# qiukunlong/seeksv

Measured on AMD Instinct MI355X. Metric: BAM records/sec through getclip+getsv, higher is better.
Workload: dtype i32/u8 (fp64 match-rate compare)

## Files before the change

include/seeksv_hip.h:

```cpp
#ifndef SEEKSV_HIP_H_
#define SEEKSV_HIP_H_

#include <stddef.h>
#include <stdint.h>

#ifdef __cplusplus
extern "C" {
#endif

#define SSV_ABI_VERSION 9

typedef enum {
	SSV_OK = 0,
	SSV_E_NODEVICE = -1,
	SSV_E_HIP = -2,
	SSV_E_ARG = -3,
	SSV_E_STATE = -4,
	SSV_E_NOMEM = -5,
	SSV_E_RANGE = -6
} ssv_status;

typedef enum {
	SSV_MEM_HOST = 0,
	SSV_MEM_DEVICE = 1,
	SSV_MEM_PERSISTENT = 2
} ssv_mem;

typedef struct {
	int32_t tid, pos;
	uint16_t flag;
	uint8_t mapq;
	uint8_t xc;
	uint16_t n_cigar;
	uint16_t pad;
	int32_t l_qseq, mtid, mpos, isize;
	uint32_t cigar_off;
	uint32_t cigar_head[5];
	uint64_t seq_off;
} ssv_record;

#define SSV_NO_SEQ UINT64_MAX
typedef struct {
	int64_t n;
	int32_t mem;
	int32_t max_ref_span;
	const int32_t *tid;
	const int32_t *pos;
	const uint16_t *flag;
	const uint8_t *mapq;
	const uint16_t *n_cigar;
	const int32_t *l_qseq;
	const int32_t *mtid;
	const int32_t *mpos;
	const int32_t *isize;
	const uint32_t *cigar_off;
	const uint32_t *cigar;
	const uint8_t *xc;
	const uint64_t *seq_off;
	const uint8_t *seqqual;
	int64_t n_cigar_total;
	int64_t seqqual_bytes;
	const ssv_record *rec;
	const uint8_t *cigar_ends;
	const struct ssv_tid_run *tid_runs;
	int64_t n_tid_runs;
} ssv_batch_t;

typedef struct ssv_tid_run { int64_t first; int32_t tid; int32_t pad; } ssv_tid_run;

typedef struct ssv_ctx ssv_ctx;


int ssv_ctx_create(int device, ssv_ctx **out);
void ssv_ctx_destroy(ssv_ctx *ctx);
int ssv_sync(ssv_ctx *ctx);
const char *ssv_last_error(const ssv_ctx *ctx);
int ssv_abi_version(void);
int ssv_device_count(void);
void *ssv_stream(ssv_ctx *ctx);

int ssv_host_alloc(size_t bytes, void **p);
int ssv_host_free(void *p);
int ssv_host_register(void *p, size_t bytes);
int ssv_host_unregister(void *p);
int ssv_host_bind_near(void *p, size_t bytes, int device);
int ssv_batch_prefetch(ssv_ctx *ctx, const ssv_batch_t *b);
int ssv_batch_prefetch_drop(ssv_ctx *ctx);

int ssv_batch_retain(ssv_ctx *ctx, const ssv_batch_t *device_batch, ssv_batch_t *out);
int ssv_batch_release(ssv_ctx *ctx, ssv_batch_t *retained);


typedef struct {
	double match_rate;
	int32_t min_mapq;
	int32_t save_low_quality;
	int32_t use_ownership;
	int32_t initial_last_tid;
	int32_t own_lo_tid, own_lo_pos;
	int32_t own_hi_tid, own_hi_pos;
} ssv_clip_params;

int ssv_clip_begin(ssv_ctx *ctx, const ssv_clip_params *p);
int ssv_clip_scan(ssv_ctx *ctx, const ssv_batch_t *b);
int ssv_clip_scan_range(ssv_ctx *ctx, const ssv_batch_t *b, int64_t rec_begin, int64_t rec_end);
int ssv_clip_event_count(ssv_ctx *ctx, int64_t *n_events);

typedef struct {
	int32_t tid;
	uint8_t side;
	uint8_t pad[3];
	int64_t first;
} ssv_table_run;

typedef struct {
	int64_t n_clusters;
	int64_t n_events;
	const int32_t *tid;
	const int32_t *pos;
	const uint8_t *side;
	const int32_t *support;
	const int32_t *left_len;
	const int32_t *right_len;
	const uint8_t *qual_missing;
	const uint64_t *str_off;
	const uint8_t *str;
	const uint64_t *cigar_off;
	const int32_t *n_cigar;
	const uint32_t *cigar;
	int32_t seq_packed;
	int32_t qual_bits;
	uint8_t qual_alphabet[64];
	int32_t format;
	int32_t base_bits;
	int32_t len_bytes, support_bytes, ncig_bytes;
	int32_t qual_group;
	const void *c_len;
	const void *c_support;
	const void *c_ncig;
	const uint8_t *c_flags;
	const ssv_table_run *runs;
	int64_t n_runs;
	const uint64_t *base_exc;
	int64_t n_base_exc;
	uint64_t str_bytes;
	uint64_t cigar_ops;
	int64_t support_sum;
	const void *c_cigar;
	int32_t cigar_bytes, pad4;
} ssv_cluster_table;

int ssv_clip_table_format(ssv_ctx *ctx, int format);
int ssv_clip_table_expand(ssv_ctx *ctx, ssv_cluster_table *t, int32_t n_threads);
typedef struct {
	int32_t narrow, pad;
	uint64_t total;
	uint64_t rows, flags, cigar, runs, base_exc, pos_esc, str;
} ssv_table_wire;
int ssv_clip_table_wire_bytes(ssv_ctx *ctx, const ssv_cluster_table *t, ssv_table_wire *out);
uint64_t ssv_table_block_bytes3(int64_t n_bases, int32_t base_bits, int32_t qual_bits);
uint64_t ssv_table_block_bytes3g(int64_t n_bases, int32_t base_bits, int32_t qual_bits, int32_t qual_group);
uint64_t ssv_table_block_bytes(int32_t left_len, int32_t right_len);

int ssv_clip_cluster(ssv_ctx *ctx, ssv_cluster_table *out);
int ssv_clip_cluster_async(ssv_ctx *ctx, int64_t *n_clusters, int64_t *n_events);
int ssv_clip_table_wait(ssv_ctx *ctx, ssv_cluster_table *out);
int ssv_clip_table_wait_prev(ssv_ctx *ctx, ssv_cluster_table *out);


int ssv_isize_begin(ssv_ctx *ctx, int32_t min_mapq, int64_t max_pairs);
int ssv_isize_accumulate(ssv_ctx *ctx, const ssv_batch_t *b, int32_t *done);
int ssv_isize_finish(ssv_ctx *ctx, int64_t *n_pairs, int32_t *mean, int32_t *sd);


typedef struct {
	int32_t up_tid;
	int32_t down_tid;
	int32_t up_pos;
	int32_t down_pos;
	int32_t beg;
	int32_t end;
	uint8_t up_strand;
	uint8_t down_strand;
	uint8_t pad[2];
} ssv_junction;

typedef struct {
	int32_t tid;
	int32_t beg;
	int32_t end;
} ssv_interval;

typedef struct {
	const ssv_junction *junctions;
	int64_t n_junctions;
	int32_t mean, sd, times;
	int32_t disc_min_mapq;
	const ssv_interval *windows;
	int64_t n_windows;
	int32_t depth_min_mapq;
	int32_t n_targets;
	const int32_t *target_len;
} ssv_getsv_params;

int ssv_getsv_begin(ssv_ctx *ctx, const ssv_getsv_params *p);
int ssv_getsv_scan(ssv_ctx *ctx, const ssv_batch_t *b);
int ssv_getsv_prime(ssv_ctx *ctx, const ssv_batch_t *b, int32_t *sufficient);
int ssv_getsv_finish(ssv_ctx *ctx, int32_t *counts,
                     const ssv_interval *ranges, int64_t n_ranges, uint64_t *range_sum,
                     const ssv_interval *points, int64_t n_points, int32_t *point_depth,
                     int32_t *max_depth);

typedef struct ssv_group ssv_group;
int ssv_group_create(ssv_ctx **ctxs, int n, ssv_group **out);
void ssv_group_destroy(ssv_group *g);
int ssv_group_uses_rccl(const ssv_group *g);
int ssv_group_allgather(ssv_group *g, int rank, const void *send, size_t bytes, void *recv);


typedef struct {
	uint64_t c_off;
	uint32_t c_len;
	uint32_t u_len;
} ssv_bgzf_block;

typedef struct {
	int64_t n_records;
	uint64_t inflated_bytes;
	uint64_t tail_offset;
	uint32_t repaired_blocks;
	int32_t last_tid;
	const uint8_t *unmapped_raw;
	uint64_t unmapped_bytes;
	uint32_t n_tid_runs;
	const uint32_t *tid_run_index;
	const int32_t *tid_run_tid;
} ssv_bamdec_info;

int ssv_bamdec_begin(ssv_ctx *ctx, int32_t n_targets, uint64_t first_record_offset);
int ssv_bamdec_target_lens(ssv_ctx *ctx, const int32_t *lens);
int ssv_bamdec_limit(ssv_ctx *ctx, uint64_t inflated_bytes);
int ssv_bamdec_expect(ssv_ctx *ctx, uint64_t inflated_bytes);
int ssv_bamdec_verify_crc(ssv_ctx *ctx, int on);
int ssv_bamdec_any_order(ssv_ctx *ctx, int on);
int ssv_bamdec_prev_tid(ssv_ctx *ctx, int32_t tid);
int ssv_bamdec_staging(ssv_ctx *ctx, int which, size_t bytes, void **host_ptr);
int ssv_bamdec_prefetch(ssv_ctx *ctx, const void *comp, size_t comp_bytes);
int ssv_bamdec_prefetch_drop(ssv_ctx *ctx);
int ssv_bamdec_decode(ssv_ctx *ctx, const void *comp, size_t comp_bytes, const ssv_bgzf_block *blocks, int64_t n_blocks, int keep_all_seq, ssv_batch_t *out);
int ssv_bamdec_last(ssv_ctx *ctx, ssv_bamdec_info *info);

typedef struct {
	int32_t mem;
	int32_t pad;
	int64_t bias;
	const char *base;
	const uint64_t *off;
	int64_t bytes;
} ssv_names_t;
int ssv_bamdec_names(ssv_ctx *ctx, ssv_names_t *out);
typedef struct {
	int32_t n_targets;
	int32_t pad;
	const char *const *target_names;
	uint64_t first_line;
} ssv_samdec_params;

typedef struct {
	int64_t n_records;
	uint64_t lines_consumed;
	uint64_t carried_bytes;
	uint64_t refused_line;
	const char *refused_reason;
} ssv_samdec_info;

int ssv_samdec_begin(ssv_ctx *ctx, const ssv_samdec_params *p);
int ssv_samdec_prefetch(ssv_ctx *ctx, const void *text, size_t bytes);
int ssv_samdec_decode(ssv_ctx *ctx, const void *text, size_t bytes, int mem, int last, ssv_batch_t *out);
int ssv_samdec_names(ssv_ctx *ctx, ssv_names_t *out);
int ssv_samdec_last(ssv_ctx *ctx, ssv_samdec_info *info);
int ssv_samdec_sorted(ssv_ctx *ctx, int keep_all_seq);
int ssv_samdec_lists(ssv_ctx *ctx, ssv_bamdec_info *out);

typedef struct {
	int64_t n, n_cigar_total, name_bytes;
	const int32_t *tid, *pos; const uint16_t *flag, *n_cigar; const uint8_t *mapq;
	const uint32_t *cigar_off, *cigar;
	const uint64_t *name_off;
	const char *names;
// ... 83 lines not shown
```

seeksv_amd/_abi.py:

```python
import ctypes as C
import os

import numpy as np

_HERE = os.path.dirname(os.path.abspath(__file__))
LIBDIR = os.environ.get("SSV_LIBDIR") or os.path.join(_HERE, "lib")

NO_SEQ = (1 << 64) - 1
MEM_HOST, MEM_DEVICE, MEM_PERSISTENT = 0, 1, 2
RECORD_DTYPE = np.dtype([("tid", np.int32), ("pos", np.int32), ("flag", np.uint16), ("mapq", np.uint8), ("xc", np.uint8), ("n_cigar", np.uint16), ("pad", np.uint16),
                         ("l_qseq", np.int32), ("mtid", np.int32), ("mpos", np.int32), ("isize", np.int32), ("cigar_off", np.uint32), ("cigar_head", np.uint32, (5,)),
                         ("seq_off", np.uint64)])
assert RECORD_DTYPE.itemsize == 64


class Batch(C.Structure):
    _fields_ = [
        ("n", C.c_int64), ("mem", C.c_int32), ("max_ref_span", C.c_int32),
        ("tid", C.c_void_p), ("pos", C.c_void_p), ("flag", C.c_void_p), ("mapq", C.c_void_p),
        ("n_cigar", C.c_void_p), ("l_qseq", C.c_void_p), ("mtid", C.c_void_p), ("mpos", C.c_void_p),
        ("isize", C.c_void_p), ("cigar_off", C.c_void_p), ("cigar", C.c_void_p), ("xc", C.c_void_p),
        ("seq_off", C.c_void_p), ("seqqual", C.c_void_p),
        ("n_cigar_total", C.c_int64), ("seqqual_bytes", C.c_int64),
        ("rec", C.c_void_p), ("cigar_ends", C.c_void_p),
# ... 241 lines not shown
        lib.ssvh_bam_open.argtypes = [C.c_char_p, C.POINTER(C.c_void_p)]
        lib.ssvh_bam_from_header.argtypes = [C.POINTER(C.c_char_p), C.POINTER(C.c_int32), C.c_int32, C.POINTER(C.c_void_p)]
        lib.ssvh_bam_close.argtypes = [C.c_void_p]
        lib.ssvh_bam_write_batch.argtypes = [C.c_char_p, C.POINTER(C.c_char_p), C.POINTER(C.c_int32), C.c_int32, C.POINTER(Batch), C.c_char_p, C.c_int64, C.c_int, C.c_int]
        lib.ssvh_bam_n_targets.argtypes = [C.c_void_p]
        lib.ssvh_bam_target_name.argtypes = [C.c_void_p, C.c_int32]
        lib.ssvh_bam_target_name.restype = C.c_char_p
        lib.ssvh_bam_target_len.argtypes = [C.c_void_p, C.c_int32]
        lib.ssvh_bam_target_len.restype = C.c_int32
        lib.ssvh_bam_read_batch.argtypes = [C.c_void_p, C.c_int64, C.c_int, C.POINTER(Batch)]
        lib.ssvh_bam_set_readahead.argtypes = [C.c_void_p, C.c_int]
        lib.ssvh_bam_raw_begin.argtypes = [C.c_void_p, C.POINTER(C.c_uint64)]
        lib.ssvh_bam_read_blocks.argtypes = [C.c_void_p, C.c_void_p, C.c_size_t, C.c_uint64, C.POINTER(BgzfBlock), C.c_int64, C.POINTER(C.c_int64), C.POINTER(C.c_size_t)]
        lib.ssvh_raw_record_fastq.argtypes = [C.c_void_p, C.c_size_t, C.c_size_t, C.POINTER(C.c_char_p), C.POINTER(C.c_char_p), C.POINTER(C.c_char_p), C.POINTER(C.c_int)]
        lib.ssvh_raw_record_fastq.restype = C.c_size_t
        lib.ssvh_bam_unmapped_count.argtypes = [C.c_void_p]
        lib.ssvh_bam_unmapped_count.restype = C.c_int64
        lib.ssvh_bam_unmapped_get.argtypes = [C.c_void_p, C.c_int64, C.POINTER(C.c_char_p), C.POINTER(C.c_char_p), C.POINTER(C.c_char_p), C.POINTER(C.c_int)]
        lib.ssvh_bam_partition.argtypes = [C.c_char_p, C.c_int32, C.c_int32, C.POINTER(BamPart)]
        lib.ssvh_bam_walk_back.argtypes = [C.c_char_p, C.c_uint64, C.c_uint32, C.c_int64, C.POINTER(C.c_uint64), C.POINTER(C.c_uint32), C.POINTER(C.c_int64)]
        lib.ssvh_bam_set_range.argtypes = [C.c_void_p, C.c_uint64, C.c_uint32, C.c_uint64, C.c_uint32]
        lib.ssvh_partition_last_error.restype = C.c_char_p
        lib.ssvh_plan_create.argtypes = [C.c_void_p, C.POINTER(JunctionIn), C.c_int64, C.POINTER(C.c_char_p), C.POINTER(C.c_int32), C.c_int64,
                                         C.c_int32, C.c_int32, C.c_int32, C.c_int32, C.POINTER(C.c_void_p)]
        lib.ssvh_plan_destroy.argtypes = [C.c_void_p]
        lib.ssvh_plan_update_isize.argtypes = [C.c_void_p, C.c_int32, C.c_int32, C.c_int32]
        for f in ("junctions", "windows", "ranges", "points"):
            fn = getattr(lib, "ssvh_plan_" + f)
            fn.argtypes = [C.c_void_p, C.POINTER(C.c_int64)]
            fn.restype = C.c_void_p
        lib.ssvh_plan_fold.argtypes = [C.c_void_p] + [C.c_void_p] * 10
        lib._typed = True
    return lib


REALIGN_HIT = [("tid", "<i4"), ("pos", "<i4"), ("q_beg", "<i4"), ("q_end", "<i4"), ("score", "<i4"), ("second", "<i4"), ("n_mismatch", "<i4"),
               ("reverse", "u1"), ("mapq", "u1"), ("pad", "u1", (2,))]
RA_F_MASKED, RA_F_OVERFLOW = 1, 2
RA_F_ALT_CUT = 4
REALIGN_GAP = [("q_at", "<i4"), ("len", "<i4")]


class RealignIndexStats(C.Structure):
    _fields_ = [("n_indexed", C.c_int64), ("n_distinct", C.c_int64), ("occ_max", C.c_int64), ("n_over_cap", C.c_int64)]


def hip_lib():
    lib = _load("libseeksv_hip.so")
    if not getattr(lib, "_typed", False):
        V = C.c_void_p
        lib.ssv_ctx_create.argtypes = [C.c_int, C.POINTER(V)]
        lib.ssv_ctx_destroy.argtypes = [V]
        lib.ssv_sync.argtypes = [V]
        lib.ssv_last_error.argtypes = [V]
        lib.ssv_last_error.restype = C.c_char_p
        lib.ssv_stream.argtypes = [V]
        lib.ssv_stream.restype = V
        lib.ssv_host_alloc.argtypes = [C.c_size_t, C.POINTER(V)]
        lib.ssv_host_free.argtypes = [V]
        lib.ssv_batch_prefetch.argtypes = [V, C.POINTER(Batch)]
        lib.ssv_batch_prefetch_drop.argtypes = [V]
        lib.ssv_clip_begin.argtypes = [V, C.POINTER(ClipParams)]
        lib.ssv_clip_scan.argtypes = [V, C.POINTER(Batch)]
        lib.ssv_clip_scan_range.argtypes = [V, C.POINTER(Batch), C.c_int64, C.c_int64]
        lib.ssv_batch_retain.argtypes = [V, C.POINTER(Batch), C.POINTER(Batch)]
        lib.ssv_batch_release.argtypes = [V, C.POINTER(Batch)]
        lib.ssv_clip_event_count.argtypes = [V, C.POINTER(C.c_int64)]
        lib.ssv_clip_cluster.argtypes = [V, C.POINTER(HipClusterTable)]
        lib.ssv_clip_table_format.argtypes = [V, C.c_int]
        lib.ssv_clip_table_expand.argtypes = [V, C.POINTER(HipClusterTable), C.c_int32]
        lib.ssv_clip_table_wire_bytes.argtypes = [V, C.POINTER(HipClusterTable), C.POINTER(TableWire)]
        lib.ssv_table_block_bytes3.argtypes = [C.c_int64, C.c_int32, C.c_int32]
        lib.ssv_table_block_bytes3.restype = C.c_uint64
        lib.ssv_table_block_bytes3g.argtypes = [C.c_int64, C.c_int32, C.c_int32, C.c_int32]
        lib.ssv_table_block_bytes3g.restype = C.c_uint64
        lib.ssv_clip_cluster_async.argtypes = [V, C.POINTER(C.c_int64), C.POINTER(C.c_int64)]
        lib.ssv_clip_table_wait.argtypes = [V, C.POINTER(HipClusterTable)]
        lib.ssv_clip_table_wait_prev.argtypes = [V, C.POINTER(HipClusterTable)]
        lib.ssv_isize_begin.argtypes = [V, C.c_int32, C.c_int64]
        lib.ssv_isize_accumulate.argtypes = [V, C.POINTER(Batch), C.POINTER(C.c_int32)]
        lib.ssv_isize_finish.argtypes = [V, C.POINTER(C.c_int64), C.POINTER(C.c_int32), C.POINTER(C.c_int32)]
        lib.ssv_getsv_begin.argtypes = [V, C.POINTER(GetsvParams)]
        lib.ssv_getsv_scan.argtypes = [V, C.POINTER(Batch)]
        lib.ssv_getsv_finish.argtypes = [V, V, V, C.c_int64, V, V, C.c_int64, V, C.POINTER(C.c_int32)]
        lib.ssv_bamdec_begin.argtypes = [V, C.c_int32, C.c_uint64]
        lib.ssv_bamdec_staging.argtypes = [V, C.c_int, C.c_size_t, C.POINTER(V)]
        lib.ssv_bamdec_decode.argtypes = [V, V, C.c_size_t, C.POINTER(BgzfBlock), C.c_int64, C.c_int, C.POINTER(Batch)]
        lib.ssv_bamdec_prefetch.argtypes = [V, V, C.c_size_t]
        lib.ssv_bamdec_prefetch_drop.argtypes = [V]
        lib.ssv_bamdec_expect.argtypes = [V, C.c_uint64]
        lib.ssv_bamdec_verify_crc.argtypes = [V, C.c_int]
        lib.ssv_host_register.argtypes = [V, C.c_size_t]
        lib.ssv_host_unregister.argtypes = [V]
        lib.ssv_bamdec_target_lens.argtypes = [V, C.POINTER(C.c_int32)]
        lib.ssv_bamdec_last.argtypes = [V, C.POINTER(BamdecInfo)]
        lib.ssv_batch_to_host.argtypes = [V, C.POINTER(Batch), C.POINTER(Batch)]
        lib.ssv_realign_index.argtypes = [V, V, C.c_int32, C.c_int64, V, C.c_int32, C.POINTER(C.c_int64)]
        lib.ssv_realign_index_sorted.argtypes = [V, V, C.c_int32, C.c_int64, V, C.c_int32, C.c_int32, C.POINTER(RealignIndexStats)]
        lib.ssv_realign_query.argtypes = [V, V, V, C.c_int64, V]
        lib.ssv_realign_query_gapped.argtypes = [V, V, V, C.c_int64, V, V]
        lib.ssv_realign_query_alts.argtypes = [V, V, V, C.c_int64, C.c_int32, C.c_int32, V, V, V, V]
        lib.ssv_realign_query_split.argtypes = [V, V, V, C.c_int64, V, V]
        lib.ssv_realign_split_batch.argtypes = [V, V, V, C.c_int64, V, V, V, V, V, C.POINTER(Batch), C.POINTER(Names)]
        lib.ssv_realign_free.argtypes = [V]
        lib.ssv_prof_enable.argtypes = [V, C.c_int]
        lib.ssv_prof_reset.argtypes = [V]
        lib.ssv_prof_get.argtypes = [V, C.c_char_p, C.POINTER(C.c_double), C.POINTER(C.c_int64), C.POINTER(C.c_int64)]
        lib.ssv_prof_names.restype = C.c_char_p
        lib.ssv_bamdec_names.argtypes = [V, C.POINTER(Names)]
        lib.ssv_bamdec_any_order.argtypes = [V, C.c_int]
        lib.ssv_rt_begin.argtypes = [V, C.POINTER(RtParams)]
        lib.ssv_rt_scan.argtypes = [V, C.POINTER(Batch), C.POINTER(Names)]
        lib.ssv_rt_finish.argtypes = [V, C.POINTER(RtResult)]
        lib.ssv_samdec_begin.argtypes = [V, C.POINTER(SamdecParams)]
        lib.ssv_samdec_prefetch.argtypes = [V, V, C.c_size_t]
        lib.ssv_samdec_decode.argtypes = [V, V, C.c_size_t, C.c_int, C.c_int, C.POINTER(Batch)]
        lib.ssv_samdec_names.argtypes = [V, C.POINTER(Names)]
        lib.ssv_samdec_last.argtypes = [V, C.POINTER(SamdecInfo)]
        lib.ssv_samdec_sorted.argtypes = [V, C.c_int]
        lib.ssv_samdec_lists.argtypes = [V, C.POINTER(BamdecInfo)]
        lib.ssv_aln_pack.argtypes = [V, C.POINTER(Batch), C.POINTER(Names), C.POINTER(AlnCols)]
        lib._typed = True
    return lib
```

seeksv_amd/csrc/bamdec_api.inc:

```

struct ssv_bamdec_state {
	int32_t n_targets = 0;
	uint64_t start = 0;
	int32_t prev_tid = 0;
	uint64_t carry = 0;
	std::vector<uint64_t> htokoff;
	uint64_t limit = UINT64_MAX;
	bool verify_crc = false;
	bool any_order = false;
	DBuf crc_tab;
	uint64_t expect_inflated = 0;
	DBuf inf_scratch, inf_dbg, tokens, tok_off, n_tok, carrybuf, comp, blocks, u_off, stream, status, chain, count, base, rec_off, stitch, small;
	TidLists tl;
	DBuf tlen; bool have_tlen = false;
	DecodedColumns cols;
	DBuf rel, stash, seq_list, raw_bytes, raw_off, raw;
	HBuf h_stage[3], h_small, h_raw[2], h_status;
	int raw_flip = 0;
	struct CompSlot {
		DBuf buf;
		const void *host = nullptr;
		size_t bytes = 0;
		hipEvent_t up = nullptr;
		hsa_signal_t up_sig{};
// ... 254 lines not shown
				HIPCHECK(c, hipMemcpyAsync(d.crc_tab.p, &h, sizeof(h), hipMemcpyHostToDevice, st));
				HIPCHECK(c, hipStreamSynchronize(st));
			}
			hipLaunchKernelGGL(ssv::k_bgzf_crc, dim3((unsigned)n_blocks), dim3(WAVE), 0, st, comp_dev, P<ssv::BgzfBlock>(d.blocks), P<uint64_t>(d.u_off), n_blocks, P<uint8_t>(d.stream),
			                   P<ssv::CrcTab>(d.crc_tab), P<int>(d.status));
		}
		if (from) { HIPCHECK(c, hipEventRecord(from->done, st)); from->read = true; from->host = nullptr; }
	}
	d.info.n_records = 0; d.info.unmapped_raw = nullptr; d.info.unmapped_bytes = 0; d.info.n_tid_runs = 0; d.info.tid_run_index = nullptr; d.info.tid_run_tid = nullptr;
	d.info.inflated_bytes = total - d.carry;
	if (n_blocks == 0) {
		if (d.carry) { c->err = "truncated BAM record"; return SSV_E_ARG; }
		return SSV_OK;
	}
	const int64_t n_units = n_blocks * ssv::UNITS_PER_BLOCK;
	CHECK(ensure_up(d.chain, (size_t)n_units * sizeof(ssv::BlockChain)));
	CHECK(ensure_up(d.rel, (size_t)((n_units + 63) / 64) * ssv::REL_CAP * 64 * 2 + 64));
	CHECK(ensure_up(d.count, (size_t)n_units * 4 + 16)); CHECK(ensure_up(d.base, (size_t)n_units * 4 + 16));
	CHECK(ensure_up(d.stitch, sizeof(ssv::StitchOut))); CHECK(ensure_up(d.small, 256));
	CHECK(ensure_host(c, d.h_small, 256)); CHECK(ensure_host(c, d.h_status, (size_t)n_blocks * 4));
	CHECK(ensure_up(c->scan_scratch, (size_t)scan_scratch_elems(std::max<int64_t>(n_units, (int64_t)(total / 36 + 1))) * 8 + 64));
	CHECK(ensure_up(c->scan_scratch64, (size_t)scan_scratch_elems((int64_t)(total / 36 + 1)) * 8 + 64));
	{
		ProfScope ps(c, P_BAM_RECORDS, n_blocks);
		hipLaunchKernelGGL(ssv::k_find_records, dim3((unsigned)((n_units + BLOCK - 1) / BLOCK)), dim3(BLOCK), 0, st, P<uint8_t>(d.stream), P<ssv::BgzfBlock>(d.blocks), P<uint64_t>(d.u_off), n_units,
		                   d.start, stream_end, d.n_targets, d.have_tlen ? P<int32_t>(d.tlen) : (const int32_t *)nullptr, P<ssv::BlockChain>(d.chain), P<uint16_t>(d.rel));
		HIPCHECK(c, hipMemsetAsync(d.stitch.p, 0, sizeof(ssv::StitchOut), st));
		hipLaunchKernelGGL(ssv::k_stitch_check, dim3((unsigned)((n_units + BLOCK - 1) / BLOCK)), dim3(BLOCK), 0, st, P<ssv::BgzfBlock>(d.blocks), P<uint64_t>(d.u_off), n_units, d.start, stream_end, P<ssv::BlockChain>(d.chain),
		                   P<uint32_t>(d.count), P<ssv::StitchOut>(d.stitch));
		hipLaunchKernelGGL(ssv::k_stitch_blocks, dim3(1), dim3(WAVE), 0, st, P<uint8_t>(d.stream), P<ssv::BgzfBlock>(d.blocks), P<uint64_t>(d.u_off), n_units, d.start, stream_end,
		                   P<ssv::BlockChain>(d.chain), P<uint32_t>(d.count), P<ssv::StitchOut>(d.stitch));
		exclusive_scan<uint32_t, uint32_t>(st, P<uint32_t>(d.count), P<uint32_t>(d.base), n_units, 0u, P<uint32_t>(c->scan_scratch), (uint32_t *)nullptr);
	}
	HIPCHECK(c, hipMemcpyAsync(d.h_small.p, d.stitch.p, sizeof(ssv::StitchOut), hipMemcpyDeviceToHost, st));
	HIPCHECK(c, hipMemcpyAsync(d.h_status.p, d.status.p, (size_t)n_blocks * 4, hipMemcpyDeviceToHost, st));
	HIPCHECK(c, hipStreamSynchronize(st));
	for (int64_t b = 0; b < n_blocks; ++b)
		if (P<int>(d.h_status)[b] != 0) {
			c->err = P<int>(d.h_status)[b] == ssv::INF_E_CRC ? "BGZF block " + std::to_string(b) + " of the chunk: CRC32 mismatch (its bytes are not what was written)"
			                                                 : "BGZF inflate failed (block " + std::to_string(b) + " of the chunk, code " + std::to_string(P<int>(d.h_status)[b]) + ")";
			return SSV_E_ARG;
		}
	const ssv::StitchOut so = *P<ssv::StitchOut>(d.h_small);
	if (so.corrupt) { c->err = "corrupt BAM record"; return SSV_E_ARG; }
	const int64_t n = so.n_records;
	d.info.n_records = n; d.info.repaired_blocks = so.n_repaired; d.info.tail_offset = so.tail;
	d.carry = stream_end - so.tail; d.start = 0;
	if (d.carry) {
		CHECK(ensure_up(d.carrybuf, (size_t)d.carry + 64));
		HIPCHECK(c, hipMemcpyAsync(d.carrybuf.p, P<uint8_t>(d.stream) + so.tail, d.carry, hipMemcpyDeviceToDevice, st));
	}
	if (n == 0) return SSV_OK;
	const size_t N = (size_t)n;
	CHECK(ensure_up(d.rec_off, N * 8 + 16));
	CHECK(d.cols.reserve(c, N, up));
	CHECK(ensure_up(d.stash, N * 8 + 16)); CHECK(ensure_up(d.seq_list, N * 4 + 16)); CHECK(ensure_up(d.raw_bytes, N * 4 + 16)); CHECK(ensure_up(d.raw_off, N * 8 + 16));
	CHECK(d.tl.reserve(c, n, up));
	HIPCHECK(c, hipMemsetAsync(d.small.p, 0, 256, st));
	uint32_t *sm = P<uint32_t>(d.small);
	{
		ProfScope ps(c, P_BAM_DECODE, n);
		hipLaunchKernelGGL(ssv::k_list_records, dim3((unsigned)((n_units + BLOCK - 1) / BLOCK)), dim3(BLOCK), 0, st, P<uint8_t>(d.stream), P<ssv::BlockChain>(d.chain), P<uint32_t>(d.count),
		                   P<uint32_t>(d.base), n_units, P<uint16_t>(d.rel), P<uint64_t>(d.rec_off));
		const ssv::RecColumns rc{P<uint32_t>(d.raw_bytes), P<uint2>(d.stash), reinterpret_cast<int32_t *>(sm), sm + 1};
		hipLaunchKernelGGL(ssv::k_record_fields, dim3((unsigned)((n + BLOCK - 1) / BLOCK)), dim3(BLOCK), 0, st, P<uint8_t>(d.stream), P<uint64_t>(d.rec_off), n, keep_all_seq, d.cols.view(), rc);
		d.cols.layout(st, n, P<uint32_t>(c->scan_scratch), P<uint64_t>(c->scan_scratch64), sm + 4, reinterpret_cast<uint64_t *>(sm + 6));
		exclusive_scan<uint32_t, uint64_t>(st, P<uint32_t>(d.raw_bytes), P<uint64_t>(d.raw_off), n, 0ull, P<uint64_t>(c->scan_scratch64), reinterpret_cast<uint64_t *>(sm + 8));
	}
	HIPCHECK(c, hipMemcpyAsync(d.h_small.p, d.small.p, 64, hipMemcpyDeviceToHost, st));
	HIPCHECK(c, hipStreamSynchronize(st));
	uint64_t seq_total, raw_total;
	const uint32_t cigar_total = P<uint32_t>(d.h_small)[4];
	memcpy(&seq_total, P<uint32_t>(d.h_small) + 6, 8); memcpy(&raw_total, P<uint32_t>(d.h_small) + 8, 8);
	if (P<uint32_t>(d.h_small)[1]) { c->err = "corrupt BAM record"; return SSV_E_ARG; }
	CHECK(d.cols.reserve_variable(c, cigar_total, (size_t)seq_total, up)); CHECK(ensure_up(d.raw, (size_t)raw_total + 64));
	const ssv::DecodedCols col = d.cols.view();
	{
		ProfScope ps(c, P_BAM_DECODE, n);
		hipLaunchKernelGGL(ssv::k_record_cigars, dim3((unsigned)((n + BLOCK * ssv::CIGARS_PER_THREAD - 1) / (BLOCK * ssv::CIGARS_PER_THREAD))), dim3(BLOCK), 0, st, P<uint8_t>(d.stream), P<uint64_t>(d.rec_off), n, col.n_cigar,
		                   col.cigar_off, P<uint2>(d.stash), col.seq_bytes, col.xc, col.seq_off, col.cigar, P<uint32_t>(d.seq_list), sm + 10);
		hipLaunchKernelGGL(ssv::k_record_seqs, dim3((unsigned)std::min<int64_t>((n * 16 + BLOCK - 1) / BLOCK, 2048)), dim3(BLOCK), 0, st, P<uint8_t>(d.stream), P<uint64_t>(d.rec_off),
		                   col.n_cigar, col.seq_bytes, col.seq_off, P<uint32_t>(d.seq_list), sm + 10, col.seqqual, col.xc);
		hipLaunchKernelGGL(ssv::k_raw_copy, dim3((unsigned)((n + BLOCK - 1) / BLOCK)), dim3(BLOCK), 0, st, P<uint8_t>(d.stream), P<uint64_t>(d.rec_off), n, P<uint32_t>(d.raw_bytes), P<uint64_t>(d.raw_off), P<uint8_t>(d.raw));
		CHECK(d.tl.launch(c, st, col.tid, col.flag, n, d.prev_tid, sm + 2, reinterpret_cast<int32_t *>(sm + 3), sm + 11));
	}
	HIPCHECK(c, hipMemcpyAsync(d.h_small.p, d.small.p, 64, hipMemcpyDeviceToHost, st));
	HIPCHECK(c, hipStreamSynchronize(st));
	const uint32_t *hs = P<uint32_t>(d.h_small);
	uint32_t n_runs = hs[2];
	if (n_runs > TidLists::RUN_CAP) {
		if (!d.any_order) { c->err = "more than 65536 contig changes in one chunk: the BAM is not coordinate sorted"; return SSV_E_ARG; }
		n_runs = 0;
	}
	d.prev_tid = (int32_t)hs[3];
	HBuf &h_raw = d.h_raw[d.raw_flip ^= 1];
	CHECK(ensure_host(c, h_raw, (size_t)raw_total + 64));
	CHECK(d.tl.fetch(c, st, n_runs));
	if (raw_total) HIPCHECK(c, hipMemcpyAsync(h_raw.p, d.raw.p, (size_t)raw_total, hipMemcpyDeviceToHost, st));
	if (n_runs || raw_total) HIPCHECK(c, hipStreamSynchronize(st));
	d.tl.changes(n_runs, d.info);
	d.info.unmapped_raw = P<uint8_t>(h_raw); d.info.unmapped_bytes = raw_total; d.info.last_tid = d.prev_tid;
	d.cols.fill(out, n, (int64_t)cigar_total, (int64_t)seq_total);
	out->max_ref_span = (int32_t)hs[0] > 0 ? (int32_t)hs[0] : 1;
	d.tl.batch_runs(hs[11], out);
	return SSV_OK;
}

int ssv_bamdec_names(ssv_ctx *c, ssv_names_t *out)
{
	if (!c || !out) return SSV_E_ARG;
	if (!c->bd) { c->err = "ssv_bamdec_names before ssv_bamdec_begin"; return SSV_E_STATE; }
	memset(out, 0, sizeof(*out));
	out->mem = SSV_MEM_DEVICE; out->bias = 36;
	out->base = P<char>(c->bd->stream); out->off = P<uint64_t>(c->bd->rec_off);
	return SSV_OK;
}

int ssv_bamdec_last(ssv_ctx *c, ssv_bamdec_info *info)
{
	if (!c || !c->bd || !info) return SSV_E_ARG;
	*info = c->bd->info;
	return SSV_OK;
}
```

seeksv_amd/csrc/bamdec_kernels.h:

```cpp
#pragma once

#include "batch_columns.h"
#include "common.h"
#include "inflate_core.h"
#include "resolve_wave.h"
#include "inflate_wave.h"

namespace ssv {

constexpr uint32_t BD_NONE = 0xffffffffu;

template <int STRIDE> struct LdsTabT {
	uint8_t *lit8; uint32_t *hi; uint8_t *dst8;
	uint8_t *len8; uint16_t *off16;
	int lane;
	static constexpr int stride = STRIDE;
	__device__ __forceinline__ uint16_t lit_get(int i) const { return (uint16_t)(lit8[i * stride + lane] | (((hi[(i >> 5) * stride + lane] >> (i & 31)) & 1u) << 8)); }
	__device__ __forceinline__ void lit_set(int i, uint16_t v)
	{
		lit8[i * stride + lane] = (uint8_t)v;
		uint32_t &w = hi[(i >> 5) * stride + lane];
		w = (w & ~(1u << (i & 31))) | ((uint32_t)(v >> 8) << (i & 31));
	}
	__device__ __forceinline__ uint16_t dst_get(int i) const { return dst8[i * stride + lane]; }
// ... 486 lines not shown
                                                        uint32_t *__restrict__ n_list)
{
	__shared__ uint32_t mine[BLOCK * CIGARS_PER_THREAD];
	__shared__ uint32_t n_mine, base;
	if (threadIdx.x == 0) n_mine = 0;
	__syncthreads();
	const int64_t i0 = (int64_t)blockIdx.x * (BLOCK * CIGARS_PER_THREAD);
	for (int t = 0; t < CIGARS_PER_THREAD; ++t) {
		const int64_t i = i0 + (int64_t)t * BLOCK + threadIdx.x;
		bool has = false;
		if (i < n) {
			const uint32_t ncig = n_cigar[i], co = cigar_off[i];
			if (ncig <= 2u) {
				const uint2 f = stash[i];
				if (ncig > 0u) cigar[co] = f.x;
				if (ncig > 1u) cigar[co + 1] = f.y;
			} else {
				const uint8_t *r = u + rec_off[i] + 4;
				const uint64_t o_cig = 32ull + r[8];
				for (uint32_t k = 0; k < ncig; ++k) cigar[co + k] = ld_u32(r + o_cig + 4ull * k);
			}
			const bool ships = seq_bytes[i] != 0u;
			if (!ships) seq_off[i] = ~0ull;
			has = ships || xc[i] == 2;
		}
		const uint64_t m = __ballot(has);
		if (m) {
			const int leader = __ffsll((long long)m) - 1;
			uint32_t at = 0;
			if (lane_id() == leader) at = atomicAdd(&n_mine, (uint32_t)__popcll(m));
			at = (uint32_t)__shfl((int)at, leader);
			if (has) mine[at + (uint32_t)__popcll(m & ((1ull << lane_id()) - 1ull))] = (uint32_t)i;
		}
	}
	__syncthreads();
	if (threadIdx.x == 0 && n_mine) base = atomicAdd(n_list, n_mine);
	__syncthreads();
	for (uint32_t k = threadIdx.x; k < n_mine; k += BLOCK) list[base + k] = mine[k];
}

__global__ __launch_bounds__(BLOCK) void k_record_seqs(const uint8_t *__restrict__ u, const uint64_t *__restrict__ rec_off, const uint16_t *__restrict__ n_cigar,
                                                      const uint32_t *__restrict__ seq_bytes, const uint64_t *__restrict__ seq_off, const uint32_t *__restrict__ list,
                                                      const uint32_t *__restrict__ n_list, uint8_t *__restrict__ seqqual, uint8_t *__restrict__ xc)
{
	const uint32_t total = *n_list;
	const int sub = (int)(threadIdx.x & 15);
	for (uint32_t e = (blockIdx.x * BLOCK + threadIdx.x) >> 4; e < total; e += gridDim.x * (BLOCK / 16)) {
		const uint32_t i = list[e];
		const uint8_t *r = u + rec_off[i] + 4;
		const uint32_t bs = ld_u32(r - 4), l_name = r[8], ncig = n_cigar[i];
		const uint64_t o_seq = 32ull + l_name + 4ull * ncig;
		const uint32_t sb = seq_bytes[i];
		if (sb) {
			const uint64_t so = seq_off[i];
			for (uint32_t k = (uint32_t)sub; k < sb; k += 16) seqqual[so + k] = r[o_seq + k];
		}
		if (sub == 0 && xc[i] == 2) {
			const int32_t l_seq = ld_i32(r + 16);
			xc[i] = (uint8_t)aux_xc_flag(r + o_seq + ((uint64_t)l_seq + 1) / 2 + (uint64_t)l_seq, r + bs);
		}
	}
}

__global__ __launch_bounds__(BLOCK) void k_raw_copy(const uint8_t *__restrict__ u, const uint64_t *__restrict__ rec_off, int64_t n, const uint32_t *__restrict__ raw_bytes,
                                                   const uint64_t *__restrict__ raw_off, uint8_t *__restrict__ raw)
{
	const int64_t i = (int64_t)blockIdx.x * BLOCK + threadIdx.x;
	const uint32_t nb = i < n ? raw_bytes[i] : 0u;
	uint64_t m = __ballot(nb != 0u);
	while (m) {
		const int l = __ffsll((long long)m) - 1;
		m &= m - 1;
		const uint32_t knb = (uint32_t)__shfl((int)nb, l);
		const int64_t ki = i - lane_id() + l;
		const uint8_t *r = u + rec_off[ki];
		const uint64_t o = raw_off[ki];
		for (uint32_t k = (uint32_t)lane_id(); k < knb; k += WAVE) raw[o + k] = r[k];
	}
}

struct TidRun { uint32_t index; int32_t tid; };
constexpr int32_t TID_NONE = INT32_MIN;

__global__ __launch_bounds__(BLOCK) void k_tid_raw_runs(const int32_t *__restrict__ tid, int64_t n, TidRun *__restrict__ runs, uint32_t cap, uint32_t *__restrict__ count)
{
	const int64_t i = (int64_t)blockIdx.x * BLOCK + threadIdx.x;
	if (i >= n) return;
	const int32_t t = tid[i];
	if (i == 0 || tid[i - 1] != t) {
		const uint32_t k = atomicAdd(count, 1u);
		if (k < cap) { runs[k].index = (uint32_t)i; runs[k].tid = t; }
	}
}


__global__ __launch_bounds__(BLOCK) void k_tid_tile_last(const int32_t *__restrict__ tid, const uint16_t *__restrict__ flag, int64_t n, int32_t *__restrict__ tile_last)
{
	__shared__ int lds[WAVES_PER_BLOCK];
	const int64_t i = (int64_t)blockIdx.x * BLOCK + threadIdx.x;
	const bool q = i < n && !(flag[i] & (F_UNMAP | F_MUNMAP));
	int idx = wave_max(q ? (int)threadIdx.x : -1);
	if (lane_id() == 0) lds[wave_id()] = idx;
	__syncthreads();
	if (threadIdx.x == 0) {
		int m = -1;
		for (int w = 0; w < WAVES_PER_BLOCK; ++w) m = lds[w] > m ? lds[w] : m;
		tile_last[blockIdx.x] = m >= 0 ? tid[(int64_t)blockIdx.x * BLOCK + m] : TID_NONE;
	}
}

__global__ __launch_bounds__(WAVE) void k_tid_tile_carry(const int32_t *__restrict__ tile_last, int64_t n_tiles, int32_t prev_tid, int32_t *__restrict__ tile_prev, int32_t *__restrict__ last_tid)
{
	int32_t cur = prev_tid;
	constexpr int AHEAD = 16;
	for (int64_t base0 = 0; base0 < n_tiles; base0 += WAVE * AHEAD) {
	int32_t vals[AHEAD];
#pragma unroll
	for (int j = 0; j < AHEAD; ++j) { const int64_t t = base0 + (int64_t)j * WAVE + lane_id(); vals[j] = t < n_tiles ? tile_last[t] : TID_NONE; }
#pragma unroll
	for (int j = 0; j < AHEAD; ++j) {
		const int64_t t = base0 + (int64_t)j * WAVE + lane_id();
		const int32_t mine = vals[j];
		const uint64_t have = __ballot(mine != TID_NONE);
		const uint64_t below = have & lanemask_lt();
		const int src = below ? 63 - __clzll((long long)below) : 0;
		const int32_t got = __shfl(mine, src, 64);
		if (t < n_tiles) tile_prev[t] = below ? got : cur;
		if (have) cur = __shfl(mine, 63 - __clzll((long long)have), 64);
	}
	}
	if (lane_id() == 0) *last_tid = cur;
}

__global__ __launch_bounds__(BLOCK) void k_tid_runs(const int32_t *__restrict__ tid, const uint16_t *__restrict__ flag, int64_t n, const int32_t *__restrict__ tile_prev,
                                                   TidRun *__restrict__ runs, uint32_t cap, uint32_t *__restrict__ n_runs)
{
	__shared__ int32_t wave_last[WAVES_PER_BLOCK];
	const int64_t i = (int64_t)blockIdx.x * BLOCK + threadIdx.x;
	const bool q = i < n && !(flag[i] & (F_UNMAP | F_MUNMAP));
	const int32_t mine = q ? tid[i] : TID_NONE;
	const uint64_t have = __ballot(q);
	const int32_t top = __shfl(mine, have ? 63 - __clzll((long long)have) : 0, 64);
	if (lane_id() == 0) wave_last[wave_id()] = have ? top : TID_NONE;
	const uint64_t below = have & lanemask_lt();
	int32_t before = __shfl(mine, below ? 63 - __clzll((long long)below) : 0, 64);
	__syncthreads();
	if (!below) {
		before = tile_prev[blockIdx.x];
		for (int w = 0; w < wave_id(); ++w) if (wave_last[w] != TID_NONE) before = wave_last[w];
	}
	if (q && mine != before) {
		const uint32_t k = atomicAdd(n_runs, 1u);
		if (k < cap) { runs[k].index = (uint32_t)i; runs[k].tid = mine; }
	}
}

}
```

seeksv_amd/csrc/getsv_api.inc:

```

struct ssv_getsv_state {
	bool active = false;
	ssv_getsv_params p{};
	std::vector<DevJunction> junc;
	std::vector<ssv_interval> win;
	std::vector<int32_t> tlen;
	std::vector<int64_t> ctg_tile_off;
	int32_t map_span = -1;
	int32_t wmax = 0;
	int64_t diff_len = 0;
	DBuf djunc, counts, wtid, wbeg, wend, woff, diff, tilemap, tile_win, tile_junc, ctgoff, maxdepth, span;
	DBuf q_tid, q_out64;
	DBuf dense_list, cap_flags, cap_deep, cap_carry, cap_ring, cap_ring_tmp, cap_tail[2][4];
	int32_t cap_tail_n = 0, cap_tail_cur = 0, cap_ring_mask = 0;
	HBuf h_q;
};

static int fill_runs(ssv_ctx *c, const ssv_batch_t *b, RunTab &R)
{
	memset(&R, 0, sizeof(R));
	if (!b->tid_runs || b->n_tid_runs <= 0 || b->n_tid_runs > RUN_MAX || getenv("SSV_NO_TID_RUNS")) return SSV_OK;
	const int64_t k = b->n_tid_runs;
	if (b->tid_runs[0].first != 0) { c->err = "tid_runs must start at record 0"; return SSV_E_ARG; }
	for (int64_t i = 0; i < k; ++i) {
		if (i && b->tid_runs[i].first <= b->tid_runs[i - 1].first) { c->err = "tid_runs must be strictly increasing"; return SSV_E_ARG; }
		if (b->tid_runs[i].first >= b->n) { c->err = "tid_runs reach past the batch"; return SSV_E_ARG; }
		R.first[i] = b->tid_runs[i].first; R.tid[i] = b->tid_runs[i].tid;
	}
	R.first[k] = b->n; R.n = (int32_t)k;
	return SSV_OK;
}

static int gs_build_tilemap(ssv_ctx *c, int32_t span)
{
	ssv_getsv_state &G = *c->getsv;
	const size_t ntile = (size_t)G.ctg_tile_off.back();
	CHECK(ensure(c, G.tilemap, ntile + 16)); CHECK(ensure(c, G.tile_win, ntile * 4 + 16)); CHECK(ensure(c, G.tile_junc, ntile * 4 + 16));
	HIPCHECK(c, hipMemsetAsync(G.tilemap.p, 0, ntile + 16, c->st));
	const int64_t nw = (int64_t)G.win.size(), nj = (int64_t)G.junc.size();
	if (nw) k_tile_mark_windows<<<grid_for(nw, BLOCK), BLOCK, 0, c->st>>>(P<int32_t>(G.wtid), P<int32_t>(G.wbeg), P<int32_t>(G.wend), nw, span, P<int64_t>(G.ctgoff),
	                                                                        G.p.n_targets, P<uint32_t>(G.tilemap), P<uint32_t>(G.tile_win));
	if (nj) k_tile_mark_junctions<<<grid_for(nj, BLOCK), BLOCK, 0, c->st>>>(P<DevJunction>(G.djunc), nj, span, G.wmax, P<int64_t>(G.ctgoff), G.p.n_targets,
	                                                                          P<uint32_t>(G.tilemap), P<uint32_t>(G.tile_junc));
	HIPCHECK(c, hipGetLastError());
	G.map_span = span;
	return SSV_OK;
}

int ssv_getsv_begin(ssv_ctx *c, const ssv_getsv_params *p)
{
	if (!c || !p || p->n_targets < 0 || p->n_junctions < 0 || p->n_windows < 0) return SSV_E_ARG;
	ssv_getsv_state &G = *c->getsv;
	if ((p->n_targets && !p->target_len) || (p->n_junctions && !p->junctions) || (p->n_windows && !p->windows)) return SSV_E_ARG;
	c->pf.clear();
	HIPCHECK(c, hipSetDevice(c->device));
	G.p = *p;
	G.tlen.assign(p->target_len, p->target_len + p->n_targets);
	G.ctg_tile_off.assign((size_t)p->n_targets + 1, 0);
	for (int t = 0; t < p->n_targets; ++t) G.ctg_tile_off[(size_t)t + 1] = G.ctg_tile_off[(size_t)t] + ((int64_t)std::max(0, G.tlen[(size_t)t]) >> TILE_SHIFT) + 1;
	G.map_span = -1;
	G.junc.clear();
	G.wmax = 0;
	for (int64_t k = 0; k < p->n_junctions; ++k) {
		const ssv_junction &s = p->junctions[k];
		DevJunction j;
		j.up_tid = s.up_tid; j.down_tid = s.down_tid; j.up_pos = s.up_pos; j.down_pos = s.down_pos; j.beg = s.beg; j.end = s.end;
		j.up_strand = s.up_strand; j.down_strand = s.down_strand; j.pad = 0; j.orig = (int32_t)k;
		G.junc.push_back(j);
		if ((int64_t)s.end - s.beg > G.wmax) G.wmax = (int32_t)std::min<int64_t>((int64_t)s.end - s.beg, 0x7fffffff);
	}
	std::stable_sort(G.junc.begin(), G.junc.end(), [](const DevJunction &a, const DevJunction &b) { return a.up_tid != b.up_tid ? a.up_tid < b.up_tid : a.beg < b.beg; });
	G.win.assign(p->windows, p->windows + p->n_windows);
	for (size_t k = 0; k < G.win.size(); ++k) {
		const ssv_interval &w = G.win[k];
		if (w.end < w.beg || (k && (G.win[k - 1].tid > w.tid || (G.win[k - 1].tid == w.tid && G.win[k - 1].end >= w.beg)))) {
			c->err = "depth windows must be sorted, disjoint and non-empty"; return SSV_E_ARG;
		}
	}
	const size_t nj = G.junc.size(), nw = G.win.size();
	std::vector<int32_t> wt(nw), wb(nw), we(nw);
	std::vector<int64_t> wo(nw + 1, 0);
	for (size_t k = 0; k < nw; ++k) { wt[k] = G.win[k].tid; wb[k] = G.win[k].beg; we[k] = G.win[k].end; wo[k + 1] = wo[k] + ((int64_t)we[k] - wb[k] + 1) + 1; }
	G.diff_len = wo[nw];
	CHECK(ensure(c, G.djunc, nj * sizeof(DevJunction) + 16)); CHECK(ensure(c, G.counts, nj * 4 + 16));
	CHECK(ensure(c, G.wtid, nw * 4 + 16)); CHECK(ensure(c, G.wbeg, nw * 4 + 16)); CHECK(ensure(c, G.wend, nw * 4 + 16)); CHECK(ensure(c, G.woff, (nw + 1) * 8));
	CHECK(ensure(c, G.diff, (size_t)G.diff_len * 4 + 16)); CHECK(ensure(c, G.ctgoff, G.ctg_tile_off.size() * 8)); CHECK(ensure(c, G.maxdepth, 16));
	CHECK(ensure(c, G.span, 16));
	if (nj) HIPCHECK(c, hipMemcpyAsync(G.djunc.p, G.junc.data(), nj * sizeof(DevJunction), hipMemcpyHostToDevice, c->st));
	if (nw) {
		HIPCHECK(c, hipMemcpyAsync(G.wtid.p, wt.data(), nw * 4, hipMemcpyHostToDevice, c->st));
		HIPCHECK(c, hipMemcpyAsync(G.wbeg.p, wb.data(), nw * 4, hipMemcpyHostToDevice, c->st));
		HIPCHECK(c, hipMemcpyAsync(G.wend.p, we.data(), nw * 4, hipMemcpyHostToDevice, c->st));
	}
	HIPCHECK(c, hipMemcpyAsync(G.woff.p, wo.data(), (nw + 1) * 8, hipMemcpyHostToDevice, c->st));
	HIPCHECK(c, hipMemcpyAsync(G.ctgoff.p, G.ctg_tile_off.data(), G.ctg_tile_off.size() * 8, hipMemcpyHostToDevice, c->st));
	HIPCHECK(c, hipMemsetAsync(G.counts.p, 0, nj * 4 + 16, c->st));
	HIPCHECK(c, hipMemsetAsync(G.diff.p, 0, (size_t)G.diff_len * 4 + 16, c->st));
	HIPCHECK(c, hipMemsetAsync(G.maxdepth.p, 0, 16, c->st));
	CHECK(ensure(c, G.cap_carry, sizeof(CapCarry))); CHECK(ensure(c, G.cap_flags, 16));
	HIPCHECK(c, hipMemsetAsync(G.cap_carry.p, 0, sizeof(CapCarry), c->st));
	G.cap_tail_n = 0; G.cap_tail_cur = 0; G.cap_ring_mask = 0;
	HIPCHECK(c, hipStreamSynchronize(c->st));
	G.active = true;
	return SSV_OK;
}

static int cap_launches(ssv_ctx *c, const GetsvArgs &a, const DevBatch &d, int64_t ntiles, int prime)
{
	ssv_getsv_state &G = *c->getsv;
	ProfScope ps(c, P_GETSV_CAND, 0);
	if (G.cap_ring_mask == 0 || (int64_t)G.map_span + 2 > (int64_t)G.cap_ring_mask + 1) {
		int64_t e = CAP_LDS_RING;
		while (e < (int64_t)G.map_span + 2) e <<= 1;
		if (e > (1ll << 30)) { c->err = "reference span of a read beyond 2^30"; return SSV_E_RANGE; }
		if (G.cap_ring_mask == 0) CHECK(ensure(c, G.cap_ring, (size_t)e * 4));
		else {
			CHECK(ensure(c, G.cap_ring_tmp, (size_t)e * 4));
			HIPCHECK(c, hipMemsetAsync(G.cap_ring_tmp.p, 0, (size_t)e * 4, c->st));
			k_cap_regrow<<<64, BLOCK, 0, c->st>>>(P<CapCarry>(G.cap_carry), P<int32_t>(G.cap_ring), G.cap_ring_mask, P<int32_t>(G.cap_ring_tmp), (int32_t)(e - 1));
			HIPCHECK(c, hipGetLastError());
			std::swap(G.cap_ring, G.cap_ring_tmp);
		}
		G.cap_ring_mask = (int32_t)(e - 1);
	}
	CHECK(ensure(c, G.cap_deep, (size_t)ntiles + 16));
	for (int s_ = 0; s_ < 2; ++s_) { CHECK(ensure(c, G.cap_tail[s_][0], CAP_TAIL * 4)); CHECK(ensure(c, G.cap_tail[s_][1], CAP_TAIL * 4)); CHECK(ensure(c, G.cap_tail[s_][2], CAP_TAIL * 4)); CHECK(ensure(c, G.cap_tail[s_][3], CAP_TAIL)); }
	CapArgs ca;
	ca.g = a; ca.span = G.map_span; ca.prime = prime;
	DBuf *ot = G.cap_tail[G.cap_tail_cur], *nt = G.cap_tail[G.cap_tail_cur ^ 1];
	ca.tail_tid = P<int32_t>(ot[0]); ca.tail_pos = P<int32_t>(ot[1]); ca.tail_end = P<int32_t>(ot[2]); ca.tail_pass = P<uint8_t>(ot[3]); ca.tail_n = G.cap_tail_n;
	ca.deep = P<uint8_t>(G.cap_deep); ca.ntiles = ntiles; ca.flags = P<int>(G.cap_flags); ca.carry = P<CapCarry>(G.cap_carry);
	ca.ring = P<int32_t>(G.cap_ring); ca.ring_mask = G.cap_ring_mask;
	ca.ntail_tid = P<int32_t>(nt[0]); ca.ntail_pos = P<int32_t>(nt[1]); ca.ntail_end = P<int32_t>(nt[2]); ca.ntail_pass = P<uint8_t>(nt[3]);
	ca.ntail_n = (int32_t)std::min<int64_t>(CAP_TAIL, (int64_t)G.cap_tail_n + d.n);
	k_cap_mark<<<(unsigned)std::min<int64_t>(ntiles, 1024), BLOCK, 0, c->st>>>(ca);
	k_cap_sweep<<<1, WAVE, 0, c->st>>>(ca);
	k_cap_tail<<<grid_for(ca.ntail_n, BLOCK), BLOCK, 0, c->st>>>(ca);
	HIPCHECK(c, hipGetLastError());
	G.cap_tail_n = ca.ntail_n; G.cap_tail_cur ^= 1;
	return SSV_OK;
}

int ssv_getsv_scan(ssv_ctx *c, const ssv_batch_t *b)
{
	if (!c || !b) return SSV_E_ARG;
	ssv_getsv_state &G = *c->getsv;
	if (!G.active) { c->err = "ssv_getsv_scan before ssv_getsv_begin"; return SSV_E_STATE; }
	HIPCHECK(c, hipSetDevice(c->device));
	if (b->n == 0) return SSV_OK;
	DevBatch d;
	CHECK(stage_batch(c, b, d));
	if (!d.cigar) { c->err = "batch without cigar"; return SSV_E_ARG; }
	int32_t span = d.max_ref_span;
	if (span <= 0) {
		HIPCHECK(c, hipMemsetAsync(G.span.p, 0, 16, c->st));
		k_max_span<<<grid_for(d.n, BLOCK), BLOCK, 0, c->st>>>(d, P<int>(G.span));
		CHECK(ensure_host(c, c->h_totals, 64));
		HIPCHECK(c, hipMemcpyAsync(c->h_totals.p, G.span.p, 4, hipMemcpyDeviceToHost, c->st));
		HIPCHECK(c, hipStreamSynchronize(c->st));
		span = std::max(1, *P<int>(c->h_totals));
	}
	if (span > G.map_span) CHECK(gs_build_tilemap(c, span));
	GetsvArgs a;
	CHECK(fill_runs(c, b, a.runs));
	static const bool verify_runs = getenv("SSV_VERIFY_RUNS") && atoi(getenv("SSV_VERIFY_RUNS")) != 0;
	if (verify_runs && a.runs.n > 0) {
		CHECK(ensure(c, c->counters, sizeof(ClipCounters)));
		CHECK(ensure_host(c, c->h_counters, sizeof(ClipCounters)));
		HIPCHECK(c, hipMemsetAsync(c->counters.p, 0, sizeof(ClipCounters), c->st));
		k_verify_runs<<<(unsigned)std::min<int64_t>(256 * 8, (d.n + BLOCK * 4 - 1) / (BLOCK * 4)), BLOCK, 0, c->st>>>(d.tid, d.n, a.runs, &P<ClipCounters>(c->counters)->n_cand);
		HIPCHECK(c, hipGetLastError());
		HIPCHECK(c, hipMemcpyAsync(c->h_counters.p, c->counters.p, sizeof(ClipCounters), hipMemcpyDeviceToHost, c->st));
		HIPCHECK(c, hipStreamSynchronize(c->st));
		const unsigned long long badrec = P<ClipCounters>(c->h_counters)->n_cand;
		if (badrec) { c->err = "tid_runs disagree with the tid column at record " + std::to_string(badrec - 1) + " (SSV_VERIFY_RUNS)"; return SSV_E_ARG; }
	}
	a.b = d; a.tilemap = P<uint8_t>(G.tilemap); a.tile_win = P<uint32_t>(G.tile_win); a.tile_junc = P<uint32_t>(G.tile_junc); a.ctg_tile_off = P<int64_t>(G.ctgoff); a.n_targets = G.p.n_targets;
	a.junc = P<DevJunction>(G.djunc); a.n_junc = (int64_t)G.junc.size(); a.junc_wmax = G.wmax;
	a.mean = G.p.mean; a.sd = G.p.sd; a.times = G.p.times; a.disc_min_mapq = G.p.disc_min_mapq;
	a.min_ins = std::max(0, a.mean - a.sd * a.times); a.max_ins = a.mean + a.sd * a.times;
	a.counts = P<int32_t>(G.counts);
	a.win_tid = P<int32_t>(G.wtid); a.win_beg = P<int32_t>(G.wbeg); a.win_end = P<int32_t>(G.wend); a.win_off = P<int64_t>(G.woff);
	a.n_win = (int64_t)G.win.size(); a.depth_min_mapq = G.p.depth_min_mapq; a.diff = P<int32_t>(G.diff);
	a.cap_flag = nullptr; a.cap_span = G.map_span;
	HIPCHECK(c, hipMemsetAsync(G.cap_flags.p, 0, 16, c->st));
	if (a.n_win > 0) a.cap_flag = P<int>(G.cap_flags);
	const int64_t ntiles = (d.n + CS_TILE - 1) / CS_TILE;
	const unsigned grid = scan_blocks(ntiles, "SSV_GETSV_SCAN_BLOCKS", 256 * 4);
	CHECK(ensure(c, c->tile_cnt, ntiles * 4));
	CHECK(ensure(c, c->tile_off, ntiles * 4));
	CHECK(ensure(c, c->counters, sizeof(ClipCounters)));
	CHECK(ensure_host(c, c->h_counters, sizeof(ClipCounters)));
	if (c->stage_cap == 0) c->stage_cap = std::max<int64_t>(1 << 16, d.n / 8);
	ClipCounters *hc = P<ClipCounters>(c->h_counters);
	ClipCounters *dc = P<ClipCounters>(c->counters);
	GetsvStage g;
	for (int attempt = 0;; ++attempt) {
		const int64_t block_cap = (c->stage_cap + grid - 1) / grid;
		CHECK(ensure(c, c->stage, (size_t)block_cap * grid * 4));
		HIPCHECK(c, hipMemsetAsync(c->counters.p, 0, sizeof(ClipCounters), c->st));
		g.tile_cnt = P<uint32_t>(c->tile_cnt); g.tile_off = P<uint32_t>(c->tile_off); g.stage = P<uint32_t>(c->stage); g.block_cap = block_cap;
		g.overflow = &dc->overflow; g.ntiles = ntiles;
		g.dense_list = nullptr; g.dense_n = nullptr; g.n_cand = &dc->n_cand;
		{
			ProfScope ps(c, P_GETSV_SCAN, d.n);
			if (a.runs.n > 0 && d.n >= CS_TILE) k_getsv_scan_runs<<<grid, BLOCK, 0, c->st>>>(a, g);
			else k_getsv_scan<<<grid, BLOCK, 0, c->st>>>(a, g);
		}
		HIPCHECK(c, hipGetLastError());
		HIPCHECK(c, hipMemcpyAsync(hc, c->counters.p, sizeof(ClipCounters), hipMemcpyDeviceToHost, c->st));
		HIPCHECK(c, hipStreamSynchronize(c->st));
		if (!hc->overflow) break;
		if (attempt > 6) { c->err = "getsv staging overflow"; return SSV_E_HIP; }
		c->stage_cap *= 4;
	}
	{
		ProfScope ps(c, P_GETSV_CAND, d.n);
		const int64_t dense_max = std::min<int64_t>(ntiles, (int64_t)(hc->n_cand / GC_DENSE_MIN));
		if (dense_max > 0) {
			CHECK(ensure(c, G.dense_list, (size_t)dense_max * sizeof(DenseTile)));
			g.dense_list = P<DenseTile>(G.dense_list); g.dense_n = P<int>(G.cap_flags) + 2;
			k_dense_tiles<<<grid_for(ntiles, BLOCK), BLOCK, 0, c->st>>>(a, g);
		}
		k_getsv_cand<<<grid_for(ntiles, WAVES_PER_BLOCK), BLOCK, 0, c->st>>>(a, g);
		if (g.dense_list) k_getsv_cand_dense<<<(unsigned)dense_max, BLOCK, 0, c->st>>>(a, g);
	}
	HIPCHECK(c, hipGetLastError());
	if (a.n_win > 0) CHECK(cap_launches(c, a, d, ntiles, 0));
	return SSV_OK;
}

int ssv_getsv_prime(ssv_ctx *c, const ssv_batch_t *b, int32_t *sufficient)
{
	if (!c || !b || !sufficient) return SSV_E_ARG;
	ssv_getsv_state &G = *c->getsv;
	if (!G.active) { c->err = "ssv_getsv_prime before ssv_getsv_begin"; return SSV_E_STATE; }
	if (G.cap_tail_n != 0) { c->err = "ssv_getsv_prime after records were scanned"; return SSV_E_STATE; }
	HIPCHECK(c, hipSetDevice(c->device));
	*sufficient = 1;
	if (b->n == 0 || G.win.empty()) return SSV_OK;
	DevBatch d;
	CHECK(stage_batch(c, b, d));
	int32_t span = d.max_ref_span;
	if (span <= 0) {
		HIPCHECK(c, hipMemsetAsync(G.span.p, 0, 16, c->st));
		k_max_span<<<grid_for(d.n, BLOCK), BLOCK, 0, c->st>>>(d, P<int>(G.span));
		CHECK(ensure_host(c, c->h_totals, 128));
		HIPCHECK(c, hipMemcpyAsync(c->h_totals.p, G.span.p, 4, hipMemcpyDeviceToHost, c->st));
		HIPCHECK(c, hipStreamSynchronize(c->st));
		span = std::max(1, *P<int>(c->h_totals));
	}
	if (span > G.map_span) CHECK(gs_build_tilemap(c, span));
	GetsvArgs a;
	memset(&a, 0, sizeof(a));
	a.b = d; a.depth_min_mapq = G.p.depth_min_mapq; a.n_targets = G.p.n_targets; a.cap_span = G.map_span;
	a.tilemap = P<uint8_t>(G.tilemap); a.tile_win = P<uint32_t>(G.tile_win); a.ctg_tile_off = P<int64_t>(G.ctgoff);
	a.win_tid = P<int32_t>(G.wtid); a.win_beg = P<int32_t>(G.wbeg); a.win_end = P<int32_t>(G.wend); a.win_off = P<int64_t>(G.woff);
	a.n_win = (int64_t)G.win.size(); a.diff = P<int32_t>(G.diff);
	int one[4] = {1, 0, 0, 0};
	HIPCHECK(c, hipMemcpyAsync(G.cap_flags.p, one, 16, hipMemcpyHostToDevice, c->st));
	HIPCHECK(c, hipStreamSynchronize(c->st));
	const int64_t ntiles = (d.n + CS_TILE - 1) / CS_TILE;
	CHECK(cap_launches(c, a, d, ntiles, 1));
	CHECK(ensure_host(c, c->h_totals, 128));
	const int64_t nt = std::min<int64_t>(ntiles, 4);
	HIPCHECK(c, hipMemcpyAsync(c->h_totals.p, G.cap_deep.p, (size_t)nt, hipMemcpyDeviceToHost, c->st));
	HIPCHECK(c, hipStreamSynchronize(c->st));
	for (int64_t t = 1; t < nt; ++t) if (P<uint8_t>(c->h_totals)[t]) *sufficient = 0;
	if (d.n < 4 * CS_TILE) *sufficient = 0;
	return SSV_OK;
}

int ssv_getsv_finish(ssv_ctx *c, int32_t *counts, const ssv_interval *ranges, int64_t n_ranges, uint64_t *range_sum,
                     const ssv_interval *points, int64_t n_points, int32_t *point_depth, int32_t *max_depth)
{
	if (!c || n_ranges < 0 || n_points < 0 || (n_ranges && (!ranges || !range_sum)) || (n_points && (!points || !point_depth))) return SSV_E_ARG;
	ssv_getsv_state &G = *c->getsv;
	if (!G.active) { c->err = "ssv_getsv_finish before ssv_getsv_begin"; return SSV_E_STATE; }
	HIPCHECK(c, hipSetDevice(c->device));
	G.active = false;
	const int64_t nw = (int64_t)G.win.size(), nj = (int64_t)G.junc.size();
	ProfScope ps(c, P_DEPTH_FINISH, nw);
	if (nw) k_depth_prefix<<<grid_for(nw, WAVES_PER_BLOCK), BLOCK, 0, c->st>>>(P<int64_t>(G.woff), nw, P<int32_t>(G.diff), P<int32_t>(G.maxdepth));
	const size_t up_bytes = ((size_t)n_ranges * 3 + (size_t)n_points * 2) * 4;
	const size_t o_pd = (size_t)n_ranges * 8, o_cnt = o_pd + (size_t)n_points * 4, o_max = o_cnt + (size_t)nj * 4, down_bytes = o_max + 4;
	CHECK(ensure_host(c, G.h_q, up_bytes + down_bytes + 64));
	CHECK(ensure(c, G.q_tid, up_bytes + 16)); CHECK(ensure(c, G.q_out64, down_bytes + 16));
	int32_t *up = P<int32_t>(G.h_q);
	uint8_t *down = P<uint8_t>(G.h_q) + ((up_bytes + 15) & ~(size_t)15);
	int32_t *rt = up, *rb = rt + n_ranges, *re = rb + n_ranges, *pt = re + n_ranges, *pb = pt + n_points;
	for (int64_t k = 0; k < n_ranges; ++k) { rt[k] = ranges[k].tid; rb[k] = ranges[k].beg; re[k] = ranges[k].end; }
	for (int64_t k = 0; k < n_points; ++k) { pt[k] = points[k].tid; pb[k] = points[k].beg; }
	int32_t *d_up = P<int32_t>(G.q_tid);
	uint8_t *d_down = P<uint8_t>(G.q_out64);
	if (up_bytes) HIPCHECK(c, hipMemcpyAsync(d_up, up, up_bytes, hipMemcpyHostToDevice, c->st));
	if (n_ranges) k_range_sum<<<grid_for(n_ranges, WAVES_PER_BLOCK), BLOCK, 0, c->st>>>(P<int32_t>(G.wtid), P<int32_t>(G.wbeg), P<int32_t>(G.wend), P<int64_t>(G.woff), nw,
	                                                                                  P<int32_t>(G.diff), d_up, d_up + n_ranges, d_up + 2 * n_ranges, n_ranges,
	                                                                                  reinterpret_cast<unsigned long long *>(d_down));
	if (n_points) k_point_depth<<<grid_for(n_points, BLOCK), BLOCK, 0, c->st>>>(P<int32_t>(G.wtid), P<int32_t>(G.wbeg), P<int32_t>(G.wend), P<int64_t>(G.woff), nw,
	                                                                          P<int32_t>(G.diff), d_up + 3 * n_ranges, d_up + 3 * n_ranges + n_points, n_points,
	                                                                          reinterpret_cast<int32_t *>(d_down + o_pd));
	if (nj) HIPCHECK(c, hipMemcpyAsync(d_down + o_cnt, G.counts.p, (size_t)nj * 4, hipMemcpyDeviceToDevice, c->st));
	HIPCHECK(c, hipMemcpyAsync(d_down + o_max, G.maxdepth.p, 4, hipMemcpyDeviceToDevice, c->st));
	HIPCHECK(c, hipGetLastError());
	HIPCHECK(c, hipMemcpyAsync(down, d_down, down_bytes, hipMemcpyDeviceToHost, c->st));
	HIPCHECK(c, hipStreamSynchronize(c->st));
	if (n_ranges) memcpy(range_sum, down, (size_t)n_ranges * 8);
	if (n_points) memcpy(point_depth, down + o_pd, (size_t)n_points * 4);
	if (counts && nj) memcpy(counts, down + o_cnt, (size_t)nj * 4);
	if (max_depth) memcpy(max_depth, down + o_max, 4);
	return SSV_OK;
// ... 2 lines not shown
```

seeksv_amd/csrc/getsv_kernels.h:

```cpp
#pragma once

#include "clip_kernels.h"
#include "common.h"

namespace ssv {

__device__ __forceinline__ bool is_hard_clip(const DevBatch &b, const RecLine &r)
{
	const int n = r.n_cigar();
	if (n == 0) return false;
	return (r.head(0) & 15u) == C_H || (r.op(b.cigar, n - 1) & 15u) == C_H;
}


constexpr int ISZ_TILE = BLOCK;

__device__ __forceinline__ bool isize_qualifies(const DevBatch &b, const RecLine &r, int min_mapq)
{
	if (r.mapq() < min_mapq) return false;
	const int f = r.flag();
	if (!((f & F_PAIRED) && (f & F_PROPER) && !(f & F_DUP))) return false;
	if (r.isize() <= 0) return false;
	return !is_hard_clip(b, r);
}

__global__ __launch_bounds__(BLOCK) void k_isize_count(DevBatch b, int min_mapq, int32_t *__restrict__ val, uint32_t *__restrict__ tile_cnt)
{
	__shared__ uint32_t lds[WAVES_PER_BLOCK];
	const int q = (int)(threadIdx.x & 3);
	uint32_t c = 0;
#pragma unroll
	for (int k = 0; k < 4; ++k) {
		const int64_t i = (int64_t)blockIdx.x * ISZ_TILE + k * (BLOCK / 4) + (threadIdx.x >> 2);
		if (i < b.n) {
			const RecLine r = rec_load_quad(b.rec, i, q);
			const bool ok = isize_qualifies(b, r, min_mapq);
			if (q == 0) { val[i] = ok ? r.isize() : 0; c += ok ? 1u : 0u; }
		}
	}
	c = wave_sum(c);
	if (lane_id() == 0) lds[wave_id()] = c;
	__syncthreads();
	if (threadIdx.x == 0) tile_cnt[blockIdx.x] = lds[0] + lds[1] + lds[2] + lds[3];
}

__global__ __launch_bounds__(BLOCK) void k_isize_first_compared(DevBatch b, int min_mapq, unsigned long long *__restrict__ first)
{
	const int64_t i = (int64_t)blockIdx.x * BLOCK + threadIdx.x;
	if (i >= b.n) return;
	const RecLine r = rec_load(b.rec, i);
	if (r.mapq() < min_mapq || is_hard_clip(b, r)) return;
	atomicMin(first, (unsigned long long)i * 2 + (isize_qualifies(b, r, min_mapq) ? 1 : 0));
}

__global__ __launch_bounds__(BLOCK) void k_isize_collect(const int32_t *__restrict__ val, int64_t n, const uint32_t *__restrict__ tile_base, int64_t count_before, int64_t max_pairs,
                                                         int32_t *__restrict__ vals)
{
	__shared__ uint32_t lds[WAVES_PER_BLOCK + 1];
	const int64_t i = (int64_t)blockIdx.x * ISZ_TILE + threadIdx.x;
	const int v = i < n ? val[i] : 0;
	uint32_t tot;
	const uint32_t ex = block_exclusive_sum(v > 0 ? 1u : 0u, lds, &tot);
	const int64_t o = count_before + tile_base[blockIdx.x] + ex;
	if (v > 0 && o < max_pairs) vals[o] = v;
}

__global__ __launch_bounds__(BLOCK) void k_isize_reduce(const int32_t *__restrict__ vals, int64_t n, int mode, const long long *__restrict__ mean_from, long long *__restrict__ acc)
{
	__shared__ long long lds[WAVES_PER_BLOCK];
	const int mean = mode ? (int)((unsigned long)*mean_from / (unsigned long)n) : 0;
	long long s = 0;
	for (int64_t i = (int64_t)blockIdx.x * blockDim.x + threadIdx.x; i < n; i += (int64_t)gridDim.x * blockDim.x) {
		int x = vals[i];
		if (mode == 0) s += x;
		else {
			int d = (int)((unsigned)x - (unsigned)mean);
			s += (int)((unsigned)d * (unsigned)d);
		}
	}
	s = wave_sum(s);
	if (lane_id() == 0) lds[wave_id()] = s;
	__syncthreads();
	if (threadIdx.x == 0) atomicAdd((unsigned long long *)acc, (unsigned long long)(lds[0] + lds[1] + lds[2] + lds[3]));
}


constexpr int TILE_SHIFT = 9;
constexpr uint8_t TM_DEPTH = 1, TM_JUNC = 2;

struct DevJunction {
	int32_t up_tid, down_tid, up_pos, down_pos, beg, end;
	uint8_t up_strand, down_strand;
	uint16_t pad;
	int32_t orig;
};

constexpr int RUN_MAX = 48;
struct RunTab {
	int32_t n;
	int32_t tid[RUN_MAX];
	int64_t first[RUN_MAX + 1];
};

struct GetsvArgs {
	DevBatch b;
	RunTab runs;
	const uint8_t *tilemap;
	const uint32_t *tile_win;
	const uint32_t *tile_junc;
	const int64_t *ctg_tile_off;
	int32_t n_targets;
	const DevJunction *junc;
	int64_t n_junc;
	int32_t junc_wmax;
	int32_t mean, sd, times, min_ins, max_ins, disc_min_mapq;
	int32_t *counts;
	const int32_t *win_tid, *win_beg, *win_end;
	const int64_t *win_off;
	int64_t n_win;
	int32_t depth_min_mapq;
	int32_t *diff;
	int *cap_flag;
	int32_t cap_span;
};

__device__ __forceinline__ bool is_concordant(int flag, int isize, int mean, int sd, int times)
{
	int lo = mean - sd * times, hi = mean + sd * times;
	if (!(flag & F_REV) && (flag & F_MREV) && lo <= isize && isize <= hi) return true;
	if ((flag & F_REV) && !(flag & F_MREV) && isize < 0) {
		int a = isize < 0 ? -isize : isize;
		return lo <= a && a <= hi;
	}
	return false;
}

__device__ __forceinline__ bool discordant_geometry(const DevJunction &j, int flag, int pos, int mpos, int lq, int mtid, int min_ins, int max_ins)
{
	if (!(j.down_tid != -1 && j.down_tid == mtid)) return false;
	const int K = 5;
	const int up = j.up_pos, down = j.down_pos;
	if (j.up_strand == '+' && j.down_strand == '+' && pos + lq <= up + K && mpos + 1 >= down - K) {
		if (!(flag & F_REV) && (flag & F_MREV)) {
			int ins = up - pos + mpos + lq - down + 1;
			if (j.up_tid == j.down_tid && up > down && up - down + 1 + 2 * lq <= max_ins) {
				while (ins <= max_ins) {
					if (ins >= min_ins) return true;
					ins += up - down + 1;
				}
				return false;
			}
			return min_ins <= ins && ins <= max_ins;
		}
		return false;
	} else if (j.up_strand == '-' && j.down_strand == '+' && (flag & F_REV) && (flag & F_MREV) && mpos + 1 >= down - K) {
		int ins = pos + 1 - up + 1 + mpos + lq - down + 1;
		return min_ins <= ins && ins <= max_ins;
	} else if (j.up_strand == '+' && j.down_strand == '-' && !(flag & F_REV) && !(flag & F_MREV) && pos + lq <= up + K && mpos + lq <= down + K) {
		int ins = up - pos + down - (mpos + lq) + 1;
		return min_ins <= ins && ins <= max_ins;
	}
	return false;
}

struct CandRec {
	int mapq, flag, isize, nc, mtid, mpos, lq;
	const uint32_t *cig;
	RecLine line;
};

__device__ __forceinline__ CandRec cand_load(const DevBatch &b, int64_t i)
{
	CandRec r;
	r.line = rec_load(b.rec, i);
	r.mapq = r.line.mapq(); r.flag = r.line.flag(); r.isize = r.line.isize(); r.nc = r.line.n_cigar(); r.mtid = r.line.mtid(); r.mpos = r.line.mpos(); r.lq = r.line.l_qseq();
	r.cig = b.cigar + r.line.cigar_off();
	return r;
}

__device__ __forceinline__ uint32_t cand_op(const CandRec &r, int k) { return k < 5 ? r.line.head(k) : r.cig[k]; }

__device__ __forceinline__ bool discordant_read(const GetsvArgs &a, const CandRec &r)
{
	if (r.mapq < a.disc_min_mapq) return false;
	const int flag = r.flag;
	if (flag & (F_DUP | F_UNMAP | F_MUNMAP)) return false;
	if (is_concordant(flag, r.isize, a.mean, a.sd, a.times)) return false;
	const int n = r.nc;
	if (n > 0 && ((cand_op(r, 0) & 15u) == C_H || (cand_op(r, n - 1) & 15u) == C_H)) return false;
	return true;
}

template <typename F, typename H> __device__ __forceinline__ void discordant_walk(const GetsvArgs &a, const CandRec &r, int tid, int pos, int64_t lo, F junction_at, H hit)
{
	const int n = r.nc;
	int rend = pos;
	if (n == 0) rend = pos + 1;
	else for (int k = 0; k < n; ++k) { const uint32_t c = cand_op(r, k); const int op = (int)(c & 15u); if (op == C_M || op == C_D || op == C_N) rend += (int)(c >> 4); }
	for (int64_t m = lo; m < a.n_junc; ++m) {
		const DevJunction j = junction_at(m);
		if (j.up_tid != tid || j.beg >= rend) break;
		if (!(rend > j.beg && pos < j.end)) continue;
		if (discordant_geometry(j, r.flag, pos, r.mpos, r.lq, r.mtid, a.min_ins, a.max_ins)) hit(m, j);
	}
}

__device__ __forceinline__ void discordant_record(const GetsvArgs &a, const CandRec &r, int tid, int pos, int64_t tile)
{
	if (!discordant_read(a, r)) return;
	discordant_walk(a, r, tid, pos, a.tile_junc[tile], [&](int64_t m) { return a.junc[m]; }, [&](int64_t, const DevJunction &j) { atomicAdd(&a.counts[j.orig], 1); });
}

__device__ __forceinline__ void depth_segment(const GetsvArgs &a, int tid, int s, int e, int64_t tile, int64_t &w, int sign)
{
	if (w < 0) w = a.tile_win[tile];
	while (w < a.n_win && a.win_tid[w] == tid && a.win_end[w] < s) ++w;
	for (int64_t x = w; x < a.n_win && a.win_tid[x] == tid && a.win_beg[x] <= e; ++x) {
		int wb = a.win_beg[x], we = a.win_end[x];
		int lo = s > wb ? s : wb, hi = e < we ? e : we;
		int32_t *d = a.diff + a.win_off[x];
		atomicAdd(&d[lo - wb], sign);
		atomicAdd(&d[hi + 1 - wb], -sign);
	}
}

__device__ __forceinline__ bool depth_counts(const GetsvArgs &a, const CandRec &r)
{
	if (r.mapq < a.depth_min_mapq) return false;
	return !(r.flag & (F_UNMAP | F_SECONDARY | F_QCFAIL | F_DUP));
}

__device__ __forceinline__ void depth_record(const GetsvArgs &a, const CandRec &r, int tid, int pos, int64_t tile, int sign = 1)
{
	if (sign > 0 && !depth_counts(a, r)) return;
	const int n = r.nc;
	int col = pos + 1;
	int64_t w = -1;
	for (int k = 0; k < n; ++k) {
		const uint32_t c = cand_op(r, k);
		int op = (int)(c & 15u), len = (int)(c >> 4);
		if (op == C_M) {
			if (len > 0) depth_segment(a, tid, col, col + len - 1, tile, w, sign);
			col += len;
		} else if (op == C_D || op == C_N) col += len;
	}
}

__device__ __forceinline__ uint32_t getsv_tile_bits(const GetsvArgs &a, int tid, int pos, int64_t &tile)
{
	tile = 0;
	if (tid < 0 || tid >= a.n_targets || pos < 0) return 0;
	int64_t t = a.ctg_tile_off[tid] + (pos >> TILE_SHIFT);
	tile = t;
	return t < a.ctg_tile_off[tid + 1] ? a.tilemap[t] : 0u;
}

__global__ void k_tile_mark_windows(const int32_t *__restrict__ win_tid, const int32_t *__restrict__ win_beg, const int32_t *__restrict__ win_end, int64_t n_win, int32_t span,
                                    const int64_t *__restrict__ ctg_tile_off, int32_t n_targets, uint32_t *__restrict__ map32, uint32_t *__restrict__ tile_win)
{
	const int64_t w = (int64_t)blockIdx.x * blockDim.x + threadIdx.x;
	if (w >= n_win) return;
	const int tid = win_tid[w];
	if (tid < 0 || tid >= n_targets) return;
	int64_t p0 = (int64_t)win_beg[w] - span, p1 = (int64_t)win_end[w] - 1;
	if (p1 < 0) return;
	if (p0 < 0) p0 = 0;
	const int64_t base = ctg_tile_off[tid], ntile = ctg_tile_off[tid + 1] - base;
	int64_t t0 = p0 >> TILE_SHIFT, t1 = p1 >> TILE_SHIFT;
	if (t0 >= ntile) return;
	if (t1 >= ntile) t1 = ntile - 1;
	for (int64_t t = t0; t <= t1; ++t) {
		const int col = (int)(t << TILE_SHIFT) + 1;
		int64_t lo = 0, hi = n_win;
		while (lo < hi) {
			const int64_t m = (lo + hi) >> 1;
			const int wt = win_tid[m];
			if (wt < tid || (wt == tid && win_end[m] < col)) lo = m + 1; else hi = m;
		}
		tile_win[base + t] = (uint32_t)lo;
		atomicOr(&map32[(base + t) >> 2], (uint32_t)TM_DEPTH << (8 * ((base + t) & 3)));
	}
}

__global__ void k_tile_mark_junctions(const DevJunction *__restrict__ junc, int64_t n_junc, int32_t span, int32_t wmax, const int64_t *__restrict__ ctg_tile_off, int32_t n_targets,
                                      uint32_t *__restrict__ map32, uint32_t *__restrict__ tile_junc)
{
	const int64_t k = (int64_t)blockIdx.x * blockDim.x + threadIdx.x;
	if (k >= n_junc) return;
	const int tid = junc[k].up_tid;
	if (tid < 0 || tid >= n_targets) return;
	int64_t p0 = (int64_t)junc[k].beg - span, p1 = (int64_t)junc[k].end - 1;
	if (p1 < 0) return;
	if (p0 < 0) p0 = 0;
	const int64_t base = ctg_tile_off[tid], ntile = ctg_tile_off[tid + 1] - base;
	int64_t t0 = p0 >> TILE_SHIFT, t1 = p1 >> TILE_SHIFT;
	if (t0 >= ntile) return;
	if (t1 >= ntile) t1 = ntile - 1;
	for (int64_t t = t0; t <= t1; ++t) {
		const int64_t want = (t << TILE_SHIFT) - (int64_t)wmax;
		int64_t lo = 0, hi = n_junc;
		while (lo < hi) {
			const int64_t m = (lo + hi) >> 1;
			if (junc[m].up_tid < tid || (junc[m].up_tid == tid && (int64_t)junc[m].beg <= want)) lo = m + 1; else hi = m;
		}
		tile_junc[base + t] = (uint32_t)lo;
		atomicOr(&map32[(base + t) >> 2], (uint32_t)TM_JUNC << (8 * ((base + t) & 3)));
	}
}

struct GetsvStage {
	uint32_t *tile_cnt, *tile_off, *stage;
	int64_t block_cap;
	int *overflow;
	int64_t ntiles;
	struct DenseTile *dense_list;
	int *dense_n;
	unsigned long long *n_cand;
};

__device__ __forceinline__ int tile_run_tid(const RunTab &R, int64_t tile, int64_t n)
{
	if (R.n <= 0 || (tile + 1) * CS_TILE > n) return -1;
	const int64_t i0 = tile * CS_TILE, i1 = (tile + 1) * CS_TILE;
	int lo = 0, hi = R.n - 1;
	while (lo < hi) { const int m = (lo + hi + 1) >> 1; if (R.first[m] <= i0) lo = m; else hi = m - 1; }
	return R.first[lo + 1] >= i1 && R.tid[lo] >= 0 ? R.tid[lo] : -1;
}

__device__ __forceinline__ void getsv_scan_load(const DevBatch &b, int64_t tile, int4 (&t4)[CS_SUB], int4 (&p4)[CS_SUB], int run_tid)
{
	const int64_t t0 = tile * CS_TILE + (int64_t)threadIdx.x * CS_ITEMS;
	if (run_tid >= 0) {
#pragma unroll
		for (int sub = 0; sub < CS_SUB; ++sub) {
			t4[sub] = make_int4(run_tid, run_tid, run_tid, run_tid);
			p4[sub] = stream_load_i4(b.pos + t0 + (int64_t)sub * (BLOCK * CS_ITEMS));
		}
	} else if ((tile + 1) * CS_TILE <= b.n) {
#pragma unroll
		for (int sub = 0; sub < CS_SUB; ++sub) {
			t4[sub] = stream_load_i4(b.tid + t0 + (int64_t)sub * (BLOCK * CS_ITEMS));
			p4[sub] = stream_load_i4(b.pos + t0 + (int64_t)sub * (BLOCK * CS_ITEMS));
		}
	} else {
#pragma unroll
		for (int sub = 0; sub < CS_SUB; ++sub) {
			const int64_t i0 = t0 + (int64_t)sub * (BLOCK * CS_ITEMS);
			int tt[CS_ITEMS], pp[CS_ITEMS];
#pragma unroll
			for (int k = 0; k < CS_ITEMS; ++k) { bool in = i0 + k < b.n; tt[k] = in ? b.tid[i0 + k] : -1; pp[k] = in ? b.pos[i0 + k] : 0; }
			t4[sub] = make_int4(tt[0], tt[1], tt[2], tt[3]); p4[sub] = make_int4(pp[0], pp[1], pp[2], pp[3]);
		}
	}
}

__global__ __launch_bounds__(BLOCK) void k_verify_runs(const int32_t *__restrict__ tid, int64_t n, RunTab runs, unsigned long long *bad)
{
	for (int64_t i0 = ((int64_t)blockIdx.x * BLOCK + threadIdx.x) * 4; i0 < n; i0 += (int64_t)gridDim.x * BLOCK * 4) {
		int k = 0;
		while (k + 1 < runs.n && runs.first[k + 1] <= i0) ++k;
		if (i0 + 4 <= n) {
			const int4 t = stream_load_i4(tid + i0);
			const int v[4] = {t.x, t.y, t.z, t.w};
#pragma unroll
			for (int j = 0; j < 4; ++j) {
				while (k + 1 < runs.n && runs.first[k + 1] <= i0 + j) ++k;
				if (v[j] != runs.tid[k]) atomicMax(bad, (unsigned long long)(i0 + j + 1));
			}
		} else for (int64_t i = i0; i < n; ++i) {
			while (k + 1 < runs.n && runs.first[k + 1] <= i) ++k;
			if (tid[i] != runs.tid[k]) atomicMax(bad, (unsigned long long)(i + 1));
		}
	}
}

__global__ __launch_bounds__(BLOCK) void k_getsv_scan(GetsvArgs a, GetsvStage g)
{
	__shared__ uint64_t lds[2][WAVES_PER_BLOCK];
	const DevBatch &b = a.b;
	uint32_t cursor = 0;
	int parity = 0;
	const int64_t region = (int64_t)blockIdx.x * g.block_cap;
	const int last_tid = a.n_targets - 1;
	int4 t4[CS_SUB], p4[CS_SUB], nt4[CS_SUB], np4[CS_SUB];
	int run = -1, nrun = -1;
	if ((int64_t)blockIdx.x < g.ntiles) { run = tile_run_tid(a.runs, blockIdx.x, b.n); getsv_scan_load(b, blockIdx.x, t4, p4, run); }
	for (int64_t tile = blockIdx.x; tile < g.ntiles; tile += gridDim.x, parity ^= 1) {
		const int64_t t0 = tile * CS_TILE + (int64_t)threadIdx.x * CS_ITEMS;
		const int64_t next = tile + gridDim.x;
		if (next < g.ntiles) { nrun = tile_run_tid(a.runs, next, b.n); getsv_scan_load(b, next, nt4, np4, nrun); }
		uint32_t mask = 0;
		const int tid0 = run >= 0 ? run : __builtin_amdgcn_readfirstlane(t4[0].x);
		bool same = true;
		int pmin = 0x7fffffff, pmax = -1;
		if (run >= 0) {
#pragma unroll
			for (int sub = 0; sub < CS_SUB; ++sub) {
				pmin = min(pmin, min(min(p4[sub].x, p4[sub].y), min(p4[sub].z, p4[sub].w)));
				pmax = max(pmax, max(max(p4[sub].x, p4[sub].y), max(p4[sub].z, p4[sub].w)));
			}
			same = pmin >= 0;
		} else {
#pragma unroll
			for (int sub = 0; sub < CS_SUB; ++sub) {
				const int tid[CS_ITEMS] = {t4[sub].x, t4[sub].y, t4[sub].z, t4[sub].w};
				const int pos[CS_ITEMS] = {p4[sub].x, p4[sub].y, p4[sub].z, p4[sub].w};
#pragma unroll
				for (int k = 0; k < CS_ITEMS; ++k) {
					same = same && tid[k] == tid0 && pos[k] >= 0;
					pmin = pos[k] < pmin ? pos[k] : pmin;
					pmax = pos[k] > pmax ? pos[k] : pmax;
				}
			}
		}
		const bool uniform = __all(same) && tid0 >= 0 && tid0 <= last_tid;
		int wmin = 0, wmax = 0;
		if (uniform) {
			const int wpmin = -wave_max(-pmin), wpmax = wave_max(pmax);
			wmin = wpmin >> TILE_SHIFT; wmax = wpmax >> TILE_SHIFT;
			if (a.cap_flag && wpmax - wpmin <= a.cap_span && lane_id() == 0) *a.cap_flag = 1;
		}
		if (uniform && wmax - wmin < WAVE) {
			const int64_t lo = scalar_load(a.ctg_tile_off + tid0), hi = scalar_load(a.ctg_tile_off + tid0 + 1);
			const int64_t mine = lo + wmin + lane_id();
			const uint64_t interesting = __ballot(mine < hi && a.tilemap[mine < hi ? mine : hi - 1] != 0);
			if (interesting) {
#pragma unroll
				for (int sub = 0; sub < CS_SUB; ++sub) {
					const int pos[CS_ITEMS] = {p4[sub].x, p4[sub].y, p4[sub].z, p4[sub].w};
#pragma unroll
					for (int k = 0; k < CS_ITEMS; ++k)
						mask |= ((uint32_t)(interesting >> ((pos[k] >> TILE_SHIFT) - wmin)) & 1u) << (sub * CS_ITEMS + k);
				}
			}
		} else {
#pragma unroll
			for (int sub = 0; sub < CS_SUB; ++sub) {
				const int tid[CS_ITEMS] = {t4[sub].x, t4[sub].y, t4[sub].z, t4[sub].w};
				const int pos[CS_ITEMS] = {p4[sub].x, p4[sub].y, p4[sub].z, p4[sub].w};
#pragma unroll
				for (int k = 0; k < CS_ITEMS; ++k) {
					const int tc = tid[k] < 0 ? 0 : (tid[k] > last_tid ? last_tid : tid[k]);
					const int64_t lo = a.ctg_tile_off[tc], hi = a.ctg_tile_off[tc + 1];
					int64_t t = lo + ((pos[k] < 0 ? 0 : pos[k]) >> TILE_SHIFT);
					const bool valid = tid[k] >= 0 && tid[k] <= last_tid && pos[k] >= 0 && t < hi;
					t = t < hi ? t : hi - 1;
					const bool cand = valid && a.tilemap[t] != 0;
					mask |= (cand ? 1u : 0u) << (sub * CS_ITEMS + k);
				}
			}
		}
		uint64_t packed = 0;
#pragma unroll
		for (int sub = 0; sub < CS_SUB; ++sub) packed |= (uint64_t)__popc((mask >> (sub * CS_ITEMS)) & ((1u << CS_ITEMS) - 1u)) << (16 * sub);
		stage_tile_candidates<CS_ITEMS, true>(mask, packed, tile, t0, lds, parity, cursor, region, g.block_cap, g.tile_cnt, g.tile_off, g.stage, g.overflow);
// ... 34 lines not shown
		uint32_t mask = 0;
#pragma nounroll
		for (int j = 0; j < CS_SUB * CS_ITEMS; ++j) {
			const int64_t i = t0 + (int64_t)(j / CS_ITEMS) * (BLOCK * CS_ITEMS) + (j % CS_ITEMS);
			const int pos = partial ? (i < b.n ? b.pos[i] : 0) : s_pos[j][threadIdx.x];
			int tid = run_;
			if (run_ < 0) {
				while (r + 1 < a.runs.n && a.runs.first[r + 1] <= i) ++r;
				tid = i < b.n ? a.runs.tid[r] : -1;
			}
			const int tc = tid < 0 ? 0 : (tid > last_tid ? last_tid : tid);
			const int64_t lo = a.ctg_tile_off[tc], hi = a.ctg_tile_off[tc + 1];
			int64_t t = lo + ((pos < 0 ? 0 : pos) >> TILE_SHIFT);
			const bool valid = tid >= 0 && tid <= last_tid && pos >= 0 && t < hi;
			t = t < hi ? t : hi - 1;
			if (valid && a.tilemap[t] != 0) mask |= 1u << j;
		}
		return mask;
	};
	constexpr int NB = CS_AHEAD + 1;
	int4 pq[NB][CS_SUB];
	int run = -1, wmin = 0, nrun = -1, nwmin = 0;
	bool fast = false, nfast = false;
	bool cap_seen = false;
	uint8_t tmq[NB];
	bool tm_in = false, ntm_in = false;
	const int full_tiles = __builtin_amdgcn_readfirstlane((int)(b.n / CS_TILE));
	auto head = [&](int64_t tile, const int4 (&q)[CS_SUB], int &run_, bool &fast_, int &wmin_, uint8_t &tm_, bool &in_) {
		run_ = tile < g.ntiles ? tile_run_tid(a.runs, tile, b.n) : -1;
		int pmin = 0x7fffffff, pmax = -1;
#pragma unroll
		for (int sub = 0; sub < CS_SUB; ++sub) {
			pmin = min(pmin, min(min(q[sub].x, q[sub].y), min(q[sub].z, q[sub].w)));
			pmax = max(pmax, max(max(q[sub].x, q[sub].y), max(q[sub].z, q[sub].w)));
		}
		const bool ok = run_ >= 0 && run_ <= last_tid && __all(pmin >= 0);
		const int wpmin = -wave_max(-pmin), wpmax = wave_max(pmax);
		wmin_ = wpmin >> TILE_SHIFT;
		cap_seen = cap_seen || (ok && wpmax - wpmin <= a.cap_span);
		fast_ = ok && (wpmax >> TILE_SHIFT) - wmin_ < WAVE;
		const int rc = ok ? run_ : 0;
		const int64_t lo = scalar_load(a.ctg_tile_off + rc), hi = scalar_load(a.ctg_tile_off + rc + 1);
		const int64_t mine = lo + (fast_ ? wmin_ : 0) + lane_id();
		in_ = fast_ && mine < hi;
		tm_ = a.tilemap[mine < hi ? mine : (hi > 0 ? hi - 1 : 0)];
	};
	auto step = [&](int64_t tile, const int4 (&cur)[CS_SUB], const int4 (&nxt)[CS_SUB], int4 (&far)[CS_SUB], const uint8_t &tm, uint8_t &ntm) {
		const int64_t t0 = tile * CS_TILE + (int64_t)threadIdx.x * CS_ITEMS;
		const int64_t next = tile + gridDim.x;
		const int ahead = (int)tile + CS_AHEAD * (int)gridDim.x;
		getsv_scan_load_pos(b, ahead < full_tiles ? ahead : full_tiles - 1, far);
		head(next, nxt, nrun, nfast, nwmin, ntm, ntm_in);
		uint32_t mask = 0;
		if (fast) {
			const uint64_t interesting = __ballot(tm_in && tm != 0);
			if (interesting) {
#pragma unroll
				for (int sub = 0; sub < CS_SUB; ++sub) {
					const int pos[CS_ITEMS] = {cur[sub].x, cur[sub].y, cur[sub].z, cur[sub].w};
#pragma unroll
					for (int k = 0; k < CS_ITEMS; ++k)
						mask |= ((uint32_t)(interesting >> ((pos[k] >> TILE_SHIFT) - wmin)) & 1u) << (sub * CS_ITEMS + k);
				}
			}
		} else mask = by_record(cur, run, tile, t0);
		uint64_t packed = 0;
#pragma unroll
		for (int sub = 0; sub < CS_SUB; ++sub) packed |= (uint64_t)__popc((mask >> (sub * CS_ITEMS)) & ((1u << CS_ITEMS) - 1u)) << (16 * sub);
		stage_tile_candidates<CS_ITEMS, true>(mask, packed, tile, t0, lds, parity, cursor, region, g.block_cap, g.tile_cnt, g.tile_off, g.stage, g.overflow);
		run = nrun; fast = nfast; wmin = nwmin; tm_in = ntm_in;
		parity ^= 1;
	};
#pragma unroll
	for (int d = 0; d < CS_AHEAD; ++d) { const int t = (int)blockIdx.x + d * (int)gridDim.x; getsv_scan_load_pos(b, t < full_tiles ? t : full_tiles - 1, pq[d]); }
	head(blockIdx.x, pq[0], run, fast, wmin, tmq[0], tm_in);
	int64_t tile = blockIdx.x;
	while (tile < g.ntiles) {
#pragma unroll
		for (int j = 0; j < NB; ++j) {
			if (tile >= g.ntiles) break;
			step(tile, pq[j], pq[(j + 1) % NB], pq[(j + CS_AHEAD) % NB], tmq[j], tmq[(j + 1) % NB]);
			tile += gridDim.x;
		}
	}
	if (g.n_cand && threadIdx.x == 0 && cursor) atomicAdd(g.n_cand, (unsigned long long)cursor);
	if (cap_seen && a.cap_flag && lane_id() == 0) *a.cap_flag = 1;
}

constexpr uint32_t GC_DENSE_MIN = 128;
constexpr int GC_COLS = 4096;

constexpr int GC_NTB = GC_COLS / (1 << TILE_SHIFT) + 1;

struct DenseTile {
	uint32_t so, n;
	int32_t T0, P0;
	int64_t tb0;
	uint32_t jlo, wlo;
	uint8_t tb[GC_NTB + 7 - (GC_NTB + 7) % 8];
};

__global__ __launch_bounds__(BLOCK) void k_dense_tiles(GetsvArgs a, GetsvStage g)
{
	__shared__ int s_w[WAVES_PER_BLOCK + 1];
	const int64_t t = (int64_t)blockIdx.x * BLOCK + threadIdx.x;
	const uint32_t n = t < g.ntiles ? g.tile_cnt[t] : 0u;
	const bool dense = n >= GC_DENSE_MIN;
	int total;
	const int at = block_exclusive_sum<int>(dense ? 1 : 0, s_w, &total);
	if (!total) return;
	if (threadIdx.x == 0) s_w[WAVES_PER_BLOCK] = atomicAdd(g.dense_n, total);
	__syncthreads();
	if (!dense) return;
	DenseTile e;
	e.so = g.tile_off[t]; e.n = n;
	const RecLine l0 = rec_load(a.b.rec, g.stage[e.so]);
	e.T0 = l0.tid(); e.P0 = l0.pos();
	e.tb0 = a.ctg_tile_off[e.T0] + (e.P0 >> TILE_SHIFT);
	const int64_t tb_end = a.ctg_tile_off[e.T0 + 1];
	int dj = -1, dd = -1;
#pragma unroll
	for (int i = GC_NTB - 1; i >= 0; --i) {
		const uint8_t m = e.tb0 + i < tb_end ? a.tilemap[e.tb0 + i] : (uint8_t)0;
		e.tb[i] = m;
		if (m & TM_JUNC) dj = i;
		if (m & TM_DEPTH) dd = i;
	}
	e.jlo = dj >= 0 ? a.tile_junc[e.tb0 + dj] : (uint32_t)a.n_junc;
	e.wlo = dd >= 0 ? a.tile_win[e.tb0 + dd] : (uint32_t)a.n_win;
	g.dense_list[s_w[WAVES_PER_BLOCK] + at] = e;
}

__global__ __launch_bounds__(BLOCK) void k_getsv_cand(GetsvArgs a, GetsvStage g)
{
	const int64_t t0 = (int64_t)blockIdx.x * WAVES_PER_BLOCK;
	uint32_t n[WAVES_PER_BLOCK], so[WAVES_PER_BLOCK], total = 0;
#pragma unroll
	for (int w = 0; w < WAVES_PER_BLOCK; ++w) {
		const bool in = t0 + w < g.ntiles;
		n[w] = in ? g.tile_cnt[t0 + w] : 0u; so[w] = in ? g.tile_off[t0 + w] : 0u;
		if (g.dense_list && n[w] >= GC_DENSE_MIN) n[w] = 0;
		total += n[w];
	}
	const uint32_t c1 = n[0], c2 = c1 + n[1], c3 = c2 + n[2];
	for (uint32_t k = threadIdx.x; k < total; k += BLOCK) {
		const uint32_t at = k < c1 ? so[0] + k : (k < c2 ? so[1] + (k - c1) : (k < c3 ? so[2] + (k - c2) : so[3] + (k - c3)));
		const CandRec r = cand_load(a.b, g.stage[at]);
		const int tid = r.line.tid(), pos = r.line.pos();
		int64_t tile;
		const uint32_t m = getsv_tile_bits(a, tid, pos, tile);
		if (m & TM_JUNC) discordant_record(a, r, tid, pos, tile);
		if (m & TM_DEPTH) depth_record(a, r, tid, pos, tile);
	}
}

constexpr int GC_JC = 32, GC_WC = 16;
constexpr int GC_U = 2;
__global__ __launch_bounds__(BLOCK) void k_getsv_cand_dense(GetsvArgs a, GetsvStage g)
{
	__shared__ int32_t s_l[GC_COLS];
	__shared__ DevJunction s_j[GC_JC];
	__shared__ int32_t s_jc[GC_JC];
	__shared__ int32_t s_wtid[GC_WC], s_wbeg[GC_WC], s_wend[GC_WC];
	__shared__ int64_t s_woff[GC_WC];
	__shared__ uint8_t s_tb[GC_NTB];
	__shared__ int32_t s_chunk[BLOCK];
// ... 346 lines not shown
```

seeksv_amd/csrc/samdec_api.inc:

```

struct ssv_samdec_state {
	enum { IDLE, ACTIVE, ENDED, FAILED } phase = IDLE;
	int32_t n_targets = 0;
	uint64_t first_line = 1, lines_done = 0, carry = 0;
	uint32_t ref_mask = 15;
	DBuf ref_slots, ref_off, ref_blob;
	DBuf text, carrybuf, tile_sep, tile_nl, sep, nlidx, small;
	DecodedColumns cols;
	DBuf name_off, rec;
	HBuf h_small;
	struct Slot { DBuf buf; const void *host = nullptr; size_t bytes = 0; hipEvent_t up = nullptr, done = nullptr; bool read = false; } slot[2];
	int next_slot = 0;
	bool have_batch = false;
	uint64_t text_bytes = 0;
	ssv_samdec_info info{};
	bool sorted = false, keep_all_seq = false, decoded = false, have_lists = false;
	int32_t prev_tid = 0;
	DBuf ship, ship_idx, seq_list, raw_bytes, raw_off, raw;
	HBuf h_raw[2];
	int raw_flip = 0;
	TidLists tl;
	ssv_bamdec_info lists{};
};

// ... 141 lines not shown
	}
	d.text_bytes = total;
	if (total == 0) {
		HIPCHECK(c, hipStreamSynchronize(st));
		d.info.carried_bytes = 0;
		if (last) d.phase = ssv_samdec_state::ENDED;
		d.have_batch = true;
		samdec_no_lists(d, bytes);
		return SSV_OK;
	}
	const int64_t len = (int64_t)total + (last ? 1 : 0), virt_at = last ? (int64_t)total : -1;
	if (last) HIPCHECK(c, hipMemsetAsync(tx + total, '\n', 1, st));
	const int64_t n_tiles = (len + ssv::SAM_TILE - 1) / ssv::SAM_TILE;
	CHECK(ensure(c, d.tile_sep, (size_t)n_tiles * 4 + 16)); CHECK(ensure(c, d.tile_nl, (size_t)n_tiles * 4 + 16));
	CHECK(ensure(c, c->scan_scratch, (size_t)scan_scratch_elems(n_tiles) * 8 + 64));
	uint32_t *sm = P<uint32_t>(d.small);
	unsigned long long *errw = P<unsigned long long>(d.small);
	HIPCHECK(c, hipMemsetAsync(d.small.p, 0, 256, st));
	HIPCHECK(c, hipMemsetAsync(d.small.p, 0xff, 8, st));
	k_sam_count<<<(unsigned)n_tiles, BLOCK, 0, st>>>(tx, len, virt_at, P<uint32_t>(d.tile_sep), P<uint32_t>(d.tile_nl));
	HIPCHECK(c, hipGetLastError());
	exclusive_scan<uint32_t, uint32_t>(st, P<uint32_t>(d.tile_sep), P<uint32_t>(d.tile_sep), n_tiles, 0u, P<uint32_t>(c->scan_scratch), sm + 2);
	exclusive_scan<uint32_t, uint32_t>(st, P<uint32_t>(d.tile_nl), P<uint32_t>(d.tile_nl), n_tiles, 0u, P<uint32_t>(c->scan_scratch), sm + 3);
	HIPCHECK(c, hipMemcpyAsync(d.h_small.p, d.small.p, 64, hipMemcpyDeviceToHost, st));
	HIPCHECK(c, hipStreamSynchronize(st));
	const uint32_t *hs = P<uint32_t>(d.h_small);
	const uint32_t n_sep = hs[2];
	const int64_t n = hs[3];
	if (n == 0) {
		CHECK(ensure(c, d.carrybuf, (size_t)total + 64));
		HIPCHECK(c, hipMemcpyAsync(d.carrybuf.p, tx, total, hipMemcpyDeviceToDevice, st));
		HIPCHECK(c, hipStreamSynchronize(st));
		d.carry = total; d.info.carried_bytes = total;
		d.have_batch = true;
		samdec_no_lists(d, bytes);
		return SSV_OK;
	}
	const size_t N = (size_t)n;
	CHECK(ensure(c, d.sep, (size_t)n_sep * 4 + 16)); CHECK(ensure(c, d.nlidx, N * 4 + 16));
	CHECK(d.cols.reserve(c, N, 1.0));
	CHECK(ensure(c, d.name_off, N * 8 + 16)); CHECK(ensure(c, d.rec, N * sizeof(ssv_record) + 64));
	CHECK(ensure(c, c->scan_scratch, (size_t)scan_scratch_elems(n) * 8 + 64)); CHECK(ensure(c, c->scan_scratch64, (size_t)scan_scratch_elems(n) * 8 + 64));
	k_sam_marks<<<(unsigned)n_tiles, BLOCK, 0, st>>>(tx, len, virt_at, P<uint32_t>(d.tile_sep), P<uint32_t>(d.tile_nl), (uint32_t)n, P<uint32_t>(d.sep), P<uint32_t>(d.nlidx), errw);
	ssv::SamSortedCols srt{};
	if (d.sorted) {
		CHECK(ensure(c, d.ship, N * 4 + 16)); CHECK(ensure(c, d.ship_idx, N * 4 + 16)); CHECK(ensure(c, d.raw_bytes, N * 4 + 16)); CHECK(ensure(c, d.raw_off, N * 8 + 16));
		CHECK(d.tl.reserve(c, n, 1.0));
		srt = ssv::SamSortedCols{P<uint32_t>(d.ship), P<uint32_t>(d.raw_bytes), P<uint32_t>(d.ship_idx), nullptr, d.keep_all_seq ? 1 : 0};
		k_sam_sizes_sorted<<<grid_for(n, BLOCK), BLOCK, 0, st>>>(tx, P<uint32_t>(d.sep), P<uint32_t>(d.nlidx), n, d.cols.view(), srt, errw);
	} else
		k_sam_sizes<<<grid_for(n, BLOCK), BLOCK, 0, st>>>(tx, P<uint32_t>(d.sep), P<uint32_t>(d.nlidx), n, d.cols.view(), errw);
	HIPCHECK(c, hipGetLastError());
	d.cols.layout(st, n, P<uint32_t>(c->scan_scratch), P<uint64_t>(c->scan_scratch64), sm + 4, reinterpret_cast<uint64_t *>(sm + 6));
	if (d.sorted) {
		exclusive_scan<uint32_t, uint32_t>(st, srt.ship, P<uint32_t>(d.ship_idx), n, 0u, P<uint32_t>(c->scan_scratch), sm + 9);
		exclusive_scan<uint32_t, uint64_t>(st, srt.raw_bytes, P<uint64_t>(d.raw_off), n, 0ull, P<uint64_t>(c->scan_scratch64), reinterpret_cast<uint64_t *>(sm + 10));
	}
	HIPCHECK(c, hipMemcpyAsync(d.h_small.p, d.small.p, 64, hipMemcpyDeviceToHost, st));
	HIPCHECK(c, hipMemcpyAsync(P<uint32_t>(d.h_small) + 16, P<uint32_t>(d.nlidx) + (n - 1), 4, hipMemcpyDeviceToHost, st));
	HIPCHECK(c, hipStreamSynchronize(st));
	unsigned long long werr;
	const uint32_t cigar_total = hs[4], last_nl_sep = hs[16];
	uint64_t seq_total;
	memcpy(&seq_total, hs + 6, 8);
	CHECK(d.cols.reserve_variable(c, cigar_total, (size_t)seq_total, 1.0));
	const uint32_t n_ship = d.sorted ? hs[9] : 0u;
	uint64_t raw_total = 0;
	if (d.sorted) {
		memcpy(&raw_total, hs + 10, 8);
		CHECK(ensure(c, d.seq_list, (size_t)n_ship * 4 + 16)); CHECK(ensure(c, d.raw, (size_t)raw_total + 64));
		srt.list = P<uint32_t>(d.seq_list);
	}
	const ssv::DecodedCols col = d.cols.view();
	const ssv::SamLineCols lines{P<uint64_t>(d.name_off), P<ssv_record>(d.rec)};
	ssv::SamRefTable T{P<uint32_t>(d.ref_slots), d.ref_mask, P<uint32_t>(d.ref_off), P<uint8_t>(d.ref_blob)};
	HIPCHECK(c, hipMemcpyAsync(P<uint32_t>(d.h_small) + 17, P<uint32_t>(d.sep) + last_nl_sep, 4, hipMemcpyDeviceToHost, st));
	if (d.sorted) {
		k_sam_fields_sorted<<<grid_for(n, BLOCK), BLOCK, 0, st>>>(tx, P<uint32_t>(d.sep), P<uint32_t>(d.nlidx), n, T, col, lines, srt, reinterpret_cast<int32_t *>(sm + 8), errw);
		if (n_ship)
			k_sam_seqqual_list<<<(unsigned)std::min<int64_t>(((int64_t)n_ship + WAVES_PER_BLOCK - 1) / WAVES_PER_BLOCK, 8192), BLOCK, 0, st>>>(tx, P<uint32_t>(d.sep), P<uint32_t>(d.nlidx), srt.list, n_ship,
			                                                                                                                                col.l_qseq, col.seq_off, col.seqqual, errw);
		if (raw_total) k_sam_raw<<<grid_for(n, BLOCK), BLOCK, 0, st>>>(tx, P<uint32_t>(d.sep), P<uint32_t>(d.nlidx), n, col, srt.raw_bytes, P<uint64_t>(d.raw_off), P<uint8_t>(d.raw), errw);
		HIPCHECK(c, hipGetLastError());
		CHECK(d.tl.launch(c, st, col.tid, col.flag, n, d.prev_tid, sm + 12, reinterpret_cast<int32_t *>(sm + 13), sm + 14));
	} else {
		k_sam_fields<<<grid_for(n, BLOCK), BLOCK, 0, st>>>(tx, P<uint32_t>(d.sep), P<uint32_t>(d.nlidx), n, T, col, lines, reinterpret_cast<int32_t *>(sm + 8), errw);
		k_sam_seqqual<<<(unsigned)std::min<int64_t>((n + WAVES_PER_BLOCK - 1) / WAVES_PER_BLOCK, 8192), BLOCK, 0, st>>>(tx, P<uint32_t>(d.sep), P<uint32_t>(d.nlidx), n, col.l_qseq, col.seq_off,
		                                                                                                                 col.seqqual, errw);
	}
	HIPCHECK(c, hipGetLastError());
	HIPCHECK(c, hipMemcpyAsync(d.h_small.p, d.small.p, 64, hipMemcpyDeviceToHost, st));
	HIPCHECK(c, hipStreamSynchronize(st));
	memcpy(&werr, d.h_small.p, 8);
	if (werr != ssv::SAM_NO_ERROR) return samdec_refuse(c, werr);
	const uint32_t n_runs = d.sorted ? hs[12] : 0u, n_raw_runs = d.sorted ? hs[14] : 0u;
	const int32_t last_tid = (int32_t)hs[13];
	if (n_runs > TidLists::RUN_CAP) {
		c->err = "more than 65536 contig changes in one chunk: the SAM text is not coordinate sorted";
		d.phase = ssv_samdec_state::FAILED;
		return SSV_E_ARG;
	}
	const uint64_t consumed = last ? total : (uint64_t)hs[17] + 1u;
	const uint64_t carry = total - consumed;
	if (carry) {
		CHECK(ensure(c, d.carrybuf, (size_t)carry + 64));
		HIPCHECK(c, hipMemcpyAsync(d.carrybuf.p, tx + consumed, carry, hipMemcpyDeviceToDevice, st));
	}
	if (d.sorted) {
		HBuf &h_raw = d.h_raw[d.raw_flip ^= 1];
		CHECK(ensure_host(c, h_raw, (size_t)raw_total + 64));
		CHECK(d.tl.fetch(c, st, n_runs));
		if (raw_total) HIPCHECK(c, hipMemcpyAsync(h_raw.p, d.raw.p, (size_t)raw_total, hipMemcpyDeviceToHost, st));
		if (carry || n_runs || raw_total) HIPCHECK(c, hipStreamSynchronize(st));
		memset(&d.lists, 0, sizeof(d.lists));
		d.prev_tid = last_tid;
		d.tl.changes(n_runs, d.lists);
		d.lists.n_records = n; d.lists.inflated_bytes = bytes; d.lists.last_tid = last_tid;
		d.lists.unmapped_raw = P<uint8_t>(h_raw); d.lists.unmapped_bytes = raw_total;
		d.have_lists = true;
	} else if (carry) HIPCHECK(c, hipStreamSynchronize(st));
	d.carry = carry;
	d.lines_done += (uint64_t)n;
	d.info.n_records = n; d.info.lines_consumed = d.lines_done; d.info.carried_bytes = carry;
	if (last) d.phase = ssv_samdec_state::ENDED;
	d.have_batch = true;
	d.cols.fill(out, n, (int64_t)cigar_total, (int64_t)seq_total);
	out->max_ref_span = (int32_t)hs[8] > 0 ? (int32_t)hs[8] : 1;
	out->rec = lines.rec;
	out->tid_runs = nullptr; out->n_tid_runs = 0;
	if (d.sorted) d.tl.batch_runs(n_raw_runs, out);
	return SSV_OK;
}

int ssv_samdec_names(ssv_ctx *c, ssv_names_t *out)
{
	if (!c || !out) return SSV_E_ARG;
	if (!c->sd || !c->sd->have_batch) { c->err = "ssv_samdec_names before a successful ssv_samdec_decode"; return SSV_E_STATE; }
	memset(out, 0, sizeof(*out));
	out->mem = SSV_MEM_DEVICE; out->bias = 0;
	out->base = P<char>(c->sd->text); out->off = P<uint64_t>(c->sd->name_off); out->bytes = (int64_t)c->sd->text_bytes;
	return SSV_OK;
}

int ssv_samdec_last(ssv_ctx *c, ssv_samdec_info *info)
{
	if (!c || !info) return SSV_E_ARG;
	if (!c->sd || c->sd->phase == ssv_samdec_state::IDLE) { c->err = "ssv_samdec_last before ssv_samdec_begin"; return SSV_E_STATE; }
	*info = c->sd->info;
	return SSV_OK;
}

int ssv_samdec_lists(ssv_ctx *c, ssv_bamdec_info *out)
{
	if (!c || !out) return SSV_E_ARG;
	if (!c->sd || !c->sd->have_lists) { c->err = "ssv_samdec_lists before a successful ssv_samdec_decode behind ssv_samdec_sorted"; return SSV_E_STATE; }
	*out = c->sd->lists;
	return SSV_OK;
}
```

seeksv_amd/csrc/seeksv_hip.hip:

```cpp
#include "seeksv_hip.h"

#include <hip/hip_runtime.h>
#include <hsa/hsa.h>
#include <hsa/hsa_ext_amd.h>
#include <dlfcn.h>
#include <sys/mman.h>
#include <sys/syscall.h>
#include <unistd.h>

#include <algorithm>
#include <chrono>
#include <condition_variable>
#include <mutex>
#include <cmath>
#include <cstdio>
#include <cstdlib>
#include <cstring>
#include <string>
#include <thread>
#include <type_traits>
#include <unordered_map>
#include <deque>
#include <functional>
#include <memory>
// ... 431 lines not shown
	double best = 0;
	for (double r : D.rate) best = std::max(best, r);
	if (rate >= 0.85 * best && rate >= 40.0) return;
	size_t next = D.cur;
	for (size_t k = 0; k < D.cand.size(); ++k) if (D.rate[k] == 0.0) { next = k; break; }
	if (next == D.cur) for (size_t k = 0; k < D.cand.size(); ++k) if (D.rate[k] > D.rate[next]) next = k;
	if (next != D.cur) {
		if (getenv("SSV_TIMING")) fprintf(stderr, "[timing] (host link: %s at %.1f GB/s on engine 0x%x: on to engine 0x%x)\n", to_host ? "to the host" : "to the device", rate, D.cand[D.cur], D.cand[next]);
		D.cur = next;
		(to_host ? L.eng_to_host : L.eng_to_device) = D.cand[next];
	} else if (best > rate) D.rate[D.cur] = rate;
	for (size_t k = 0; k < D.cand.size(); ++k) if (k != D.cur && D.rate[k] > 0.0) D.rate[k] = std::max(rate, D.rate[k] * 0.9);
}


int ensure_host(ssv_ctx *c, HBuf &b, size_t bytes)
{
	if (bytes <= b.cap) return SSV_OK;
	size_t ncap = (std::max(bytes, b.cap + b.cap / 2) + 255) & ~(size_t)255;
	HIPCHECK(c, b.release());
	HIPCHECK(c, pinned_new(&b.p, ncap, hipHostMallocDefault));
	b.cap = ncap;
	return SSV_OK;
}

int arena_alloc(ssv_ctx *c, Arena &a, size_t bytes, void **out)
{
	bytes = (bytes + 255) & ~(size_t)255;
	while (a.cur < a.chunks.size() && a.chunks[a.cur].cap - a.used < bytes) { ++a.cur; a.used = 0; }
	if (a.cur == a.chunks.size()) {
		DBuf b;
		const size_t cap = std::max<size_t>(bytes, (size_t)64 << 20);
		HIPCHECK(c, dev_malloc(c, &b.p, cap));
		b.cap = cap;
		a.chunks.push_back(std::move(b));
		a.used = 0;
	}
	*out = reinterpret_cast<uint8_t *>(a.chunks[a.cur].p) + a.used;
	a.used += bytes;
	return SSV_OK;
}

template <typename T> T *P(DBuf &b) { return reinterpret_cast<T *>(b.p); }
template <typename T> T *P(HBuf &b) { return reinterpret_cast<T *>(b.p); }

inline size_t grown(size_t bytes, double grow) { return grow > 1.0 ? (size_t)((double)bytes * grow) + 64 : bytes; }

struct DecodedColumns {
	DBuf col[COL_COUNT], seq_bytes;
	int reserve(ssv_ctx *c, size_t n, double grow)
	{
		for (int k = 0; k < COL_COUNT; ++k) if (kBatchCols[k].len == LEN_N) CHECK(ensure(c, col[k], grown(n * kBatchCols[k].elem + 16, grow)));
		return ensure(c, seq_bytes, grown(n * 4 + 16, grow));
	}
	int reserve_variable(ssv_ctx *c, size_t cigar_total, size_t seq_total, double grow)
	{
		CHECK(ensure(c, col[COL_cigar], grown(cigar_total * 4 + 64, grow)));
		return ensure(c, col[COL_seqqual], grown(seq_total + 64, grow));
	}
	DecodedCols view()
	{
		DecodedCols v;
#define X(member, ...) v.member = static_cast<decltype(v.member)>(col[COL_##member].p);
		SSV_BATCH_COLUMNS(X)
#undef X
		v.seq_bytes = P<uint32_t>(seq_bytes);
		return v;
	}
	void layout(hipStream_t st, int64_t n, uint32_t *scratch32, uint64_t *scratch64, uint32_t *cigar_total, uint64_t *seq_total)
	{
		const DecodedCols v = view();
		exclusive_scan<uint16_t, uint32_t>(st, v.n_cigar, v.cigar_off, n, 0u, scratch32, cigar_total);
		exclusive_scan<uint32_t, uint64_t>(st, v.seq_bytes, v.seq_off, n, 0ull, scratch64, seq_total);
	}
	void fill(ssv_batch_t *out, int64_t n, int64_t cigar_total, int64_t seq_total)
	{
		out->n = n; out->n_cigar_total = cigar_total; out->seqqual_bytes = seq_total;
		for (int k = 0; k < COL_COUNT; ++k) col_set(*out, k, col[k].p);
	}
};

struct TidLists {
	static constexpr uint32_t RUN_CAP = 1u << 16, RAW_RUN_CAP = 64;
	DBuf tile_last, tile_prev, runs, raw_runs;
	HBuf h_raw_runs, h_runs;
	std::vector<ssv_tid_run> tid_runs;
	int reserve(ssv_ctx *c, int64_t n, double grow)
	{
		const size_t n_tiles = (size_t)((n + BLOCK - 1) / BLOCK);
		CHECK(ensure(c, tile_last, grown(n_tiles * 4, grow))); CHECK(ensure(c, tile_prev, grown(n_tiles * 4, grow)));
		CHECK(ensure(c, runs, grown((size_t)RUN_CAP * sizeof(ssv::TidRun), grow)));
		CHECK(ensure(c, raw_runs, grown((size_t)RAW_RUN_CAP * sizeof(ssv::TidRun), grow)));
		return ensure_host(c, h_raw_runs, (size_t)RAW_RUN_CAP * sizeof(ssv::TidRun));
	}
	int launch(ssv_ctx *c, hipStream_t st, const int32_t *tid, const uint16_t *flag, int64_t n, int32_t prev_tid, uint32_t *n_runs, int32_t *last_tid, uint32_t *n_raw_runs)
	{
		const int64_t n_tiles = (n + BLOCK - 1) / BLOCK;
		hipLaunchKernelGGL(ssv::k_tid_tile_last, dim3((unsigned)n_tiles), dim3(BLOCK), 0, st, tid, flag, n, P<int32_t>(tile_last));
		hipLaunchKernelGGL(ssv::k_tid_tile_carry, dim3(1), dim3(WAVE), 0, st, P<int32_t>(tile_last), n_tiles, prev_tid, P<int32_t>(tile_prev), last_tid);
		hipLaunchKernelGGL(ssv::k_tid_runs, dim3((unsigned)n_tiles), dim3(BLOCK), 0, st, tid, flag, n, P<int32_t>(tile_prev), P<ssv::TidRun>(runs), RUN_CAP, n_runs);
		hipLaunchKernelGGL(ssv::k_tid_raw_runs, dim3((unsigned)n_tiles), dim3(BLOCK), 0, st, tid, n, P<ssv::TidRun>(raw_runs), RAW_RUN_CAP, n_raw_runs);
		HIPCHECK(c, hipMemcpyAsync(h_raw_runs.p, raw_runs.p, (size_t)RAW_RUN_CAP * sizeof(ssv::TidRun), hipMemcpyDeviceToHost, st));
		return SSV_OK;
	}
	int fetch(ssv_ctx *c, hipStream_t st, uint32_t n_runs)
	{
		CHECK(ensure_host(c, h_runs, (size_t)n_runs * sizeof(ssv::TidRun) + 64 + (size_t)n_runs * 8));
		if (n_runs) HIPCHECK(c, hipMemcpyAsync(h_runs.p, runs.p, (size_t)n_runs * sizeof(ssv::TidRun), hipMemcpyDeviceToHost, st));
		return SSV_OK;
	}
	void changes(uint32_t n_runs, ssv_bamdec_info &info)
	{
		ssv::TidRun *r = P<ssv::TidRun>(h_runs);
		std::sort(r, r + n_runs, [](const ssv::TidRun &a, const ssv::TidRun &b) { return a.index < b.index; });
		uint32_t *idx = reinterpret_cast<uint32_t *>(P<uint8_t>(h_runs) + (((size_t)n_runs * sizeof(ssv::TidRun) + 63) & ~(size_t)63));
		int32_t *tv = reinterpret_cast<int32_t *>(idx + n_runs);
		for (uint32_t k = 0; k < n_runs; ++k) { idx[k] = r[k].index; tv[k] = r[k].tid; }
		info.n_tid_runs = n_runs; info.tid_run_index = idx; info.tid_run_tid = tv;
	}
	void batch_runs(uint32_t nr, ssv_batch_t *out)
	{
		tid_runs.clear();
		if (nr < 1 || nr > RAW_RUN_CAP) return;
		const ssv::TidRun *r = P<ssv::TidRun>(h_raw_runs);
		for (uint32_t k = 0; k < nr; ++k) tid_runs.push_back(ssv_tid_run{(int64_t)r[k].index, r[k].tid, 0});
		std::sort(tid_runs.begin(), tid_runs.end(), [](const ssv_tid_run &a, const ssv_tid_run &b) { return a.first < b.first; });
		out->tid_runs = tid_runs.data(); out->n_tid_runs = (int64_t)nr;
	}
};

int check_names(ssv_ctx *c, const ssv_names_t *nm, int64_t n, const char *what)
{
	const char *bad = nullptr;
	if (n > 0 && (!nm || !nm->base || !nm->off)) bad = "a batch with records needs their names";
	else if (nm && nm->mem != SSV_MEM_HOST && nm->mem != SSV_MEM_DEVICE) bad = "bad names.mem";
	else if (nm && nm->bias < 0) bad = "names.bias below 0";
	else if (nm && nm->mem == SSV_MEM_HOST && nm->bytes < 0) bad = "names.bytes below 0";
	if (!bad) return SSV_OK;
	c->err = std::string(what) + ": " + bad;
	return SSV_E_ARG;
}

int stage_names(ssv_ctx *c, const ssv_names_t *nm, int64_t n, DBuf &blob, DBuf &off, DevNames &out)
{
	if (nm->mem == SSV_MEM_DEVICE) { out = DevNames{nm->base, nm->off, nm->bias}; return SSV_OK; }
	CHECK(ensure(c, blob, (size_t)nm->bytes + 16)); CHECK(ensure(c, off, (size_t)n * 8 + 16));
	if (nm->bytes) HIPCHECK(c, hipMemcpyAsync(blob.p, nm->base, (size_t)nm->bytes, hipMemcpyHostToDevice, c->st));
	HIPCHECK(c, hipMemsetAsync(P<char>(blob) + nm->bytes, 0, 16, c->st));
	HIPCHECK(c, hipMemcpyAsync(off.p, nm->off, (size_t)n * 8, hipMemcpyHostToDevice, c->st));
	out = DevNames{P<char>(blob), P<uint64_t>(off), nm->bias};
	return SSV_OK;
}

struct ProfScope {
	ssv_ctx *c;
	int id;
	bool on;
	hipEvent_t a{}, b{};
	int64_t units;
	ProfScope(ssv_ctx *ctx, int id_, int64_t units_) : c(ctx), id(id_), units(units_)
	{
		on = c->prof_mode == 1 || (c->prof_mode == 2 && (id == P_CLIP_SCAN || id == P_GETSV_SCAN));
		if (!on) return;
		for (hipEvent_t *e : {&a, &b}) {
			if (!c->prof_pool.empty()) { *e = c->prof_pool.back(); c->prof_pool.pop_back(); }
			else if (hipEventCreate(e) != hipSuccess) { on = false; return; }
		}
		(void)hipEventRecord(a, c->st);
	}
	~ProfScope()
	{
		if (!on) return;
		(void)hipEventRecord(b, c->st);
		c->prof_recs.push_back({id, a, b, units});
	}
};

void prof_collect(ssv_ctx *c)
{
	if (c->prof_recs.empty()) return;
	(void)hipStreamSynchronize(c->st);
	for (ProfRec &r : c->prof_recs) {
		float ms = 0;
		if (hipEventElapsedTime(&ms, r.a, r.b) == hipSuccess) {
			c->prof_ms[r.id] += ms; c->prof_launches[r.id] += 1; c->prof_units[r.id] += r.units;
		}
		c->prof_pool.push_back(r.a); c->prof_pool.push_back(r.b);
	}
	c->prof_recs.clear();
}

inline unsigned scan_blocks(int64_t ntiles, const char *env, int64_t dflt)
{
	const char *e = getenv(env);
	int64_t cfg = e ? atoll(e) : dflt;
	return (unsigned)std::max<int64_t>(1, std::min<int64_t>(ntiles, std::min<int64_t>(cfg, CS_MAX_BLOCKS)));
}

inline unsigned grid_for(int64_t n, int per_block) { return (unsigned)std::max<int64_t>(1, (n + per_block - 1) / per_block); }

bool aligned16(const void *p) { return (reinterpret_cast<uintptr_t>(p) & 15) == 0; }
bool aligned64(const void *p) { return (reinterpret_cast<uintptr_t>(p) & 63) == 0; }

static int upload_host_batch(ssv_ctx *c, const ssv_batch_t *b, int set, hipStream_t st)
{
	const size_t n = (size_t)b->n;
	ssv_ctx::StageSet &S = c->ss[set];
	for (int k = 0; k < COL_COUNT; ++k) {
		const void *src = b->rec && kBatchCols[k].in_rec ? nullptr : col_get(*b, k);
// ... 400 lines not shown
```

seeksv_amd/device.py:

```python
import ctypes as C

import numpy as np

from . import _abi
from .host import concat_tables, host_tid_runs, table_to_dict


class SeeksvError(RuntimeError):
    pass


class Context:

    def __init__(self, device=0):
        self._lib = _abi.hip_lib()
        h = C.c_void_p()
        rc = self._lib.ssv_ctx_create(device, C.byref(h))
        if rc != 0:
            raise SeeksvError(f"ssv_ctx_create({device}) failed ({rc}): {self._lib.ssv_last_error(None).decode()}")
        self._h = h
        self.device = device

    def _check(self, rc, what):
        if rc != 0:
# ... 240 lines not shown
        return n.value

    def clip_cluster(self, as_dict=True):
        t = _abi.HipClusterTable()
        self._check(self._lib.ssv_clip_cluster(self._h, C.byref(t)), "ssv_clip_cluster")
        return table_to_dict(t) if as_dict else t

    def clip_cluster_async(self):
        nc, ne = C.c_int64(), C.c_int64()
        self._check(self._lib.ssv_clip_cluster_async(self._h, C.byref(nc), C.byref(ne)), "ssv_clip_cluster_async")
        return nc.value, ne.value

    def clip_table_wait(self, prev=False, as_dict=False):
        t = _abi.HipClusterTable()
        fn = self._lib.ssv_clip_table_wait_prev if prev else self._lib.ssv_clip_table_wait
        self._check(fn(self._h, C.byref(t)), "ssv_clip_table_wait")
        return table_to_dict(t) if as_dict else t

    def clip_table_expand(self, t, n_threads=0):
        self._check(self._lib.ssv_clip_table_expand(self._h, C.byref(t), int(n_threads)), "ssv_clip_table_expand")
        return t

    def clip_table_wire_bytes(self, t):
        w = _abi.TableWire()
        self._check(self._lib.ssv_clip_table_wire_bytes(self._h, C.byref(t), C.byref(w)), "ssv_clip_table_wire_bytes")
        return {k: int(getattr(w, k)) for k, _ in _abi.TableWire._fields_ if k != "pad"}

    def clip_scan_range(self, batch, rec_begin, rec_end):
        b, keep = self._as_batch(batch)
        self._check(self._lib.ssv_clip_scan_range(self._h, C.byref(b), int(rec_begin), int(rec_end)), "ssv_clip_scan_range")

    def getclip(self, batches, match_rate=0.9, min_mapq=1, save_low_quality=False, own=None, initial_last_tid=0, tid_runs=None):
        tables = []
        self.clip_begin(match_rate, min_mapq, save_low_quality, own, initial_last_tid)
        last_tid = pass_max = int(initial_last_tid)
        for bi, b in enumerate(batches):
            runs = tid_runs[bi] if tid_runs is not None else (host_tid_runs(b, last_tid) if isinstance(b, dict) and b.get("flag") is not None else [])
            n = len(b["tid"]) if isinstance(b, dict) else int(b.n)
            lo = 0
            for i, tid in runs:
                if tid <= pass_max and own is None:
                    self.clip_scan_range(b, lo, i)
                    tables.append(self.clip_cluster())
                    self.clip_begin(match_rate, min_mapq, save_low_quality, own, last_tid)
                    lo, pass_max = i, tid
                pass_max = max(pass_max, tid)
                last_tid = tid
            self.clip_scan_range(b, lo, n)
        tables.append(self.clip_cluster())
        return tables[0] if len(tables) == 1 else concat_tables(tables)

    def isize_stats(self, batches, min_mapq=20, max_pairs=5000000):
        self._check(self._lib.ssv_isize_begin(self._h, min_mapq, max_pairs), "ssv_isize_begin")
        done = C.c_int32(0)
        for bt in batches:
            b, keep = self._as_batch(bt)
            self._check(self._lib.ssv_isize_accumulate(self._h, C.byref(b), C.byref(done)), "ssv_isize_accumulate")
            if done.value:
                break
        n, mean, sd = C.c_int64(), C.c_int32(0), C.c_int32(0)
        self._check(self._lib.ssv_isize_finish(self._h, C.byref(n), C.byref(mean), C.byref(sd)), "ssv_isize_finish")
        return (1 if n.value == 0 else 0), n.value, mean.value, sd.value

    def getsv_begin(self, junctions, windows, mean, sd, target_lens, times=4, disc_min_mapq=20, depth_min_mapq=20):
        j = np.ascontiguousarray(junctions, dtype=_abi.JUNCTION_DTYPE)
        w = np.ascontiguousarray(windows, dtype=_abi.INTERVAL_DTYPE)
        tl = np.ascontiguousarray(target_lens, dtype=np.int32)
        p = _abi.GetsvParams()
        p.junctions = j.ctypes.data if len(j) else None
        p.n_junctions = len(j)
        p.mean, p.sd, p.times, p.disc_min_mapq = mean, sd, times, disc_min_mapq
        p.windows = w.ctypes.data if len(w) else None
        p.n_windows = len(w)
        p.depth_min_mapq = depth_min_mapq
        p.n_targets = len(tl)
        p.target_len = tl.ctypes.data if len(tl) else None
        self._gs_nj = len(j)
        self._check(self._lib.ssv_getsv_begin(self._h, C.byref(p)), "ssv_getsv_begin")

    def getsv_scan(self, batch):
        b, keep = self._as_batch(batch)
        self._check(self._lib.ssv_getsv_scan(self._h, C.byref(b)), "ssv_getsv_scan")

    def getsv_finish(self, ranges, points):
        r = np.ascontiguousarray(ranges, dtype=_abi.INTERVAL_DTYPE)
        q = np.ascontiguousarray(points, dtype=_abi.INTERVAL_DTYPE)
        counts = np.zeros(self._gs_nj, dtype=np.int32)
        rs = np.zeros(len(r), dtype=np.uint64)
        pd = np.zeros(len(q), dtype=np.int32)
        mx = C.c_int32(0)
        ptr = lambda a: a.ctypes.data if a.size else None
        self._check(self._lib.ssv_getsv_finish(self._h, ptr(counts), ptr(r), len(r), ptr(rs), ptr(q), len(q), ptr(pd), C.byref(mx)), "ssv_getsv_finish")
        return counts, rs, pd, mx.value

    def discordant_and_depth(self, batches, plan, mean, sd, min_mapq, target_lens):
        self.getsv_begin(plan.junctions, plan.windows, mean, sd, target_lens, 4, min_mapq, min_mapq)
        for b in batches:
            self.getsv_scan(b)
        counts, rs, pd, _ = self.getsv_finish(plan.ranges, plan.points)
        return counts, rs, pd

    def realign_index(self, ref2bit, target_off, mem=_abi.MEM_HOST):
        off = np.ascontiguousarray(target_off, np.int64)
        ptr = ref2bit.ctypes.data if isinstance(ref2bit, np.ndarray) else int(ref2bit)
        dropped = C.c_int64()
        self._check(self._lib.ssv_realign_index(self._h, ptr, mem, int(off[-1]), off.ctypes.data, len(off) - 1, C.byref(dropped)), "ssv_realign_index")
        return dropped.value

    def realign_index_sorted(self, ref2bit, target_off, max_occ, mem=_abi.MEM_HOST):
        off = np.ascontiguousarray(target_off, np.int64)
        ptr = ref2bit.ctypes.data if isinstance(ref2bit, np.ndarray) else int(ref2bit)
        st = _abi.RealignIndexStats()
        self._check(self._lib.ssv_realign_index_sorted(self._h, ptr, mem, int(off[-1]), off.ctypes.data, len(off) - 1, int(max_occ), C.byref(st)), "ssv_realign_index_sorted")
        return {k: int(getattr(st, k)) for k, _ in st._fields_}

    @staticmethod
    def _realign_io(seqs):
        off = np.concatenate([[0], np.cumsum([len(x) for x in seqs])]).astype(np.uint64)
        return "".join(seqs).encode(), off, np.zeros(len(seqs), dtype=np.dtype(_abi.REALIGN_HIT))

    def realign(self, seqs, gapped=False):
        blob, off, hits = self._realign_io(seqs)
        if not gapped:
            if len(seqs):
                self._check(self._lib.ssv_realign_query(self._h, C.c_char_p(blob), off.ctypes.data, len(seqs), hits.ctypes.data), "ssv_realign_query")
            return hits
        gaps = np.zeros(len(seqs), dtype=np.dtype(_abi.REALIGN_GAP))
        if len(seqs):
            self._check(self._lib.ssv_realign_query_gapped(self._h, C.c_char_p(blob), off.ctypes.data, len(seqs), hits.ctypes.data, gaps.ctypes.data), "ssv_realign_query_gapped")
        return hits, gaps

    def realign_alts(self, seqs, max_alt, gapped=False):
        n = len(seqs)
        blob, off, hits = self._realign_io(seqs)
        gaps = np.zeros(n, dtype=np.dtype(_abi.REALIGN_GAP)) if gapped else None
        alt_off = np.full(n + 1, -1, dtype=np.int64)
        alts = np.zeros(max(n * max(int(max_alt), 0), 1), dtype=np.dtype(_abi.REALIGN_HIT))
        self._check(self._lib.ssv_realign_query_alts(self._h, C.c_char_p(blob), off.ctypes.data, n, int(max_alt), 1 if gapped else 0, hits.ctypes.data,
                                                     gaps.ctypes.data if gapped else None, alt_off.ctypes.data, alts.ctypes.data), "ssv_realign_query_alts")
        return hits, gaps, alt_off, alts[:int(alt_off[n])].copy()

    def realign_split(self, seqs):
        n = len(seqs)
        blob, off, hits = self._realign_io(seqs)
        mates = np.zeros(max(n, 1), dtype=np.dtype(_abi.REALIGN_HIT))
        self._check(self._lib.ssv_realign_query_split(self._h, C.c_char_p(blob), off.ctypes.data, n, hits.ctypes.data, mates.ctypes.data), "ssv_realign_query_split")
        return hits, mates[:n]

    def realign_split_batch(self, seqs, names, quals=None):
        n = len(seqs)
        if len(names) != n or (quals is not None and [len(x) for x in quals] != [len(x) for x in seqs]):
            raise ValueError("realign_split_batch: one name per read, qualities as long as their reads")
        blob, off, hits = self._realign_io(seqs)
        mates = np.zeros(max(n, 1), dtype=np.dtype(_abi.REALIGN_HIT))
        hits = hits if n else np.zeros(1, dtype=np.dtype(_abi.REALIGN_HIT))
        raw = [x.encode() if isinstance(x, str) else bytes(x) for x in names]
        nblob = b"".join(x + b"\0" for x in raw)
        noff = np.concatenate([[0], np.cumsum([len(x) + 1 for x in raw])]).astype(np.uint64)
        qblob = C.c_char_p("".join(quals).encode()) if quals is not None else None
        b, nm = _abi.Batch(), _abi.Names()
        self._check(self._lib.ssv_realign_split_batch(self._h, C.c_char_p(blob), off.ctypes.data, n, qblob, C.c_char_p(nblob), noff.ctypes.data, hits.ctypes.data,
                                                      mates.ctypes.data, C.byref(b), C.byref(nm)), "ssv_realign_split_batch")
        return hits[:n], mates[:n], b, nm

    def prof_enable(self, mode=1):
        self._check(self._lib.ssv_prof_enable(self._h, mode), "ssv_prof_enable")
# ... 47 lines not shown
```

seeksv_amd/synth.py:

```python
import ctypes as C
import math
import os

import numpy as np

from . import _abi

HG38 = [248956422, 242193529, 198295559, 190214555, 181538259, 170805979, 159345973, 145138636, 138394717, 133797422, 135086622,
        133275309, 114364328, 107043718, 101991189, 90338345, 83257441, 80373285, 58617616, 64444167, 46709983, 50818468, 156040895, 57227415]
HG38_NAMES = [f"chr{i}" for i in range(1, 23)] + ["chrX", "chrY"]
SEED = 0x5EE45F
MAX_CONTIGS = 64


class SyConfig(C.Structure):
    _fields_ = [("seed", C.c_uint64), ("n_total", C.c_int64), ("n_contigs", C.c_int32), ("read_len", C.c_int32),
                ("contig_off", C.c_int64 * (MAX_CONTIGS + 1)), ("contig_len", C.c_int32 * MAX_CONTIGS), ("spacing_fp", C.c_uint64),
                ("clip_permille", C.c_int32), ("indel_permille", C.c_int32), ("dup_permille", C.c_int32), ("sec_permille", C.c_int32),
                ("improper_permille", C.c_int32), ("vaf_permille", C.c_int32), ("n_breakends", C.c_int32), ("qual_model", C.c_int32), ("unmap_permille", C.c_int32)]


BREAKEND_DTYPE = np.dtype([("lin", np.int64), ("tid", np.int32), ("q", np.int32), ("ptid", np.int32), ("ppos", np.int32),
                           ("side", np.int8), ("pdir", np.int8), ("mate_rev", np.int8), ("is_up", np.int8), ("mate_anchor", np.int32)])
assert BREAKEND_DTYPE.itemsize == 32
# ... 189 lines not shown
            out = np.zeros(n_words, np.uint64)
            lib.ssvs_ref_2bit(C.byref(self.cfg), C.c_void_p(out.ctypes.data), C.c_int64(n_words))
            return out, off
        import torch
        lib = _lib(True)
        torch.cuda.set_device(device)
        out = torch.zeros(n_words, dtype=torch.int64, device=torch.device("cuda", device))
        if lib.ssvs_ref_2bit(C.byref(self.cfg), C.c_void_p(out.data_ptr()), C.c_int64(n_words)) != 0:
            raise RuntimeError("ssvs_ref_2bit: " + lib.ssvs_last_error().decode())
        return out, off

    def generate_host(self, g0, n, with_rec=False, all_seq=False):
        lib = _lib(False)
        be = self.breakends
        bep = be.ctypes.data if len(be) else None
        a = dict(n_cigar=np.zeros(n, np.uint16), cigar_off=np.zeros(n, np.uint32), seq_off=np.zeros(n, np.uint64))
        nct, sqb = C.c_int64(), C.c_int64()
        p = lambda x: x.ctypes.data if x.size else None
        lib.ssvs_plan(C.byref(self.cfg), bep, g0, n, p(a["n_cigar"]), p(a["cigar_off"]), p(a["seq_off"]), C.byref(nct), C.byref(sqb))
        for name, dt in (("tid", np.int32), ("pos", np.int32), ("flag", np.uint16), ("mapq", np.uint8), ("l_qseq", np.int32),
                         ("mtid", np.int32), ("mpos", np.int32), ("isize", np.int32)):
            a[name] = np.zeros(n, dt)
        a["cigar"] = np.zeros(nct.value, np.uint32)
        a["seqqual"] = np.zeros(sqb.value, np.uint8)
        rec = np.zeros(n, _abi.RECORD_DTYPE) if with_rec else None
        a["cigar_ends"] = np.zeros(n, np.uint8)
        lib.ssvs_fill(C.byref(self.cfg), bep, g0, n, p(a["tid"]), p(a["pos"]), p(a["flag"]), p(a["mapq"]), p(a["n_cigar"]), p(a["l_qseq"]),
                      p(a["mtid"]), p(a["mpos"]), p(a["isize"]), p(a["cigar_off"]), p(a["cigar"]), p(a["seq_off"]), p(a["seqqual"]),
                      p(rec) if with_rec else None, p(a["cigar_ends"]))
        if with_rec:
            a["rec"] = rec
        if all_seq:
            entry = (self.read_len + 1) // 2 + self.read_len
            a["seqqual"] = np.empty(n * entry + 16, np.uint8)
            a["seq_off"] = (np.arange(n, dtype=np.uint64) * np.uint64(entry))
            lib.ssvs_fill_seq_all(C.byref(self.cfg), bep, C.c_int64(g0), C.c_int64(n), p(a["seqqual"]))
            a["seqqual_bytes"] = n * entry
        a["xc"] = None
        a["max_ref_span"] = self.max_ref_span
        return a

    def generate_device(self, g0, n, device, soa=True, persistent=False):
        import torch
        lib = _lib(True)
        torch.cuda.set_device(device)
        dev = torch.device("cuda", device)
        if device not in self._be_dev:
            be = self.breakends
            self._be_dev[device] = torch.from_numpy(be.view(np.uint8).copy()).to(dev) if len(be) else torch.zeros(32, dtype=torch.uint8, device=dev)
        bep = self._be_dev[device].data_ptr()
        t = dict(n_cigar=torch.empty(n, dtype=torch.int16, device=dev), cigar_off=torch.empty(n, dtype=torch.int32, device=dev),
                 seq_off=torch.empty(n, dtype=torch.int64, device=dev))
        nct, sqb = C.c_int64(), C.c_int64()
        torch.cuda.synchronize(dev)
        rc = lib.ssvs_plan(C.byref(self.cfg), bep, g0, n, t["n_cigar"].data_ptr(), t["cigar_off"].data_ptr(), t["seq_off"].data_ptr(), C.byref(nct), C.byref(sqb))
        if rc != 0:
            raise RuntimeError("ssvs_plan: " + lib.ssvs_last_error().decode())
        cold = (("flag", torch.int16), ("mapq", torch.uint8), ("l_qseq", torch.int32), ("mtid", torch.int32), ("mpos", torch.int32), ("isize", torch.int32))
        for name, dt in (("tid", torch.int32), ("pos", torch.int32)) + (cold if soa else ()):
            t[name] = torch.empty(n, dtype=dt, device=dev)
        t["cigar"] = torch.empty(max(nct.value, 4), dtype=torch.int32, device=dev)
        t["seqqual"] = torch.empty(sqb.value + 16, dtype=torch.uint8, device=dev)
        t["rec"] = torch.empty(max(n, 1) * 64, dtype=torch.uint8, device=dev)
        t["cigar_ends"] = torch.empty(n + 16, dtype=torch.uint8, device=dev)
        ptr = lambda k: t[k].data_ptr() if k in t else None
        rc = lib.ssvs_fill(C.byref(self.cfg), bep, g0, n, ptr("tid"), ptr("pos"), ptr("flag"), ptr("mapq"),
                           ptr("n_cigar"), ptr("l_qseq"), ptr("mtid"), ptr("mpos"), ptr("isize"),
                           ptr("cigar_off"), ptr("cigar"), ptr("seq_off"), ptr("seqqual"), ptr("rec"), ptr("cigar_ends"))
        if rc != 0:
            raise RuntimeError("ssvs_fill: " + lib.ssvs_last_error().decode())
        if not soa:
            del t["cigar_off"], t["seq_off"]
        arrays = {k: v.data_ptr() for k, v in t.items()}
        arrays["xc"] = None
        arrays["n_cigar_total"] = nct.value
        arrays["seqqual_bytes"] = sqb.value
        arrays["max_ref_span"] = self.max_ref_span
        if n > 1:
            tt = t["tid"]
            ch = (torch.nonzero(tt[1:] != tt[:-1]).flatten() + 1).cpu().numpy()
            starts = np.concatenate(([0], ch)).astype(np.int64)
            runs = np.zeros(len(starts), _abi.TID_RUN_DTYPE)
            runs["first"], runs["tid"] = starts, tt[torch.from_numpy(starts).to(dev)].cpu().numpy()
            arrays["tid_runs"] = runs
        elif n == 1:
            runs = np.zeros(1, _abi.TID_RUN_DTYPE)
            runs["tid"] = int(t["tid"][0].item())
            arrays["tid_runs"] = runs
        b, _ = _abi.make_batch(arrays, mem=_abi.MEM_DEVICE | (_abi.MEM_PERSISTENT if persistent else 0), n=n)
        return b, t
```

Before: 68.78 billion.

## Skip getsv scan tiles via position-sorted tid runs and compacted tile list

Tid runs now carry a 'position-sorted' flag, computed on device during decode by counting pos descents and in the synth path on the host. When every run is sorted, getsv first builds a per-tile sub-block mask from the pos endpoints against the marked tilemap. It compacts the tiles that still need work into a list, and a new list-driven scan kernel visits only those tiles instead of streaming every record. This adds two small pre-pass kernels plus extra work in decode and validation, and it relies on the sortedness flag being correct.

```diff
diff --git a/include/seeksv_hip.h b/include/seeksv_hip.h
--- a/include/seeksv_hip.h
+++ b/include/seeksv_hip.h
@@ -66,7 +66,7 @@
 	int64_t n_tid_runs;
 } ssv_batch_t;
 
-typedef struct ssv_tid_run { int64_t first; int32_t tid; int32_t pad; } ssv_tid_run;
+typedef struct ssv_tid_run { int64_t first; int32_t tid; int32_t pad;  } ssv_tid_run;
 
 typedef struct ssv_ctx ssv_ctx;
 
@@ -205,6 +205,7 @@
 
 int ssv_getsv_begin(ssv_ctx *ctx, const ssv_getsv_params *p);
 int ssv_getsv_scan(ssv_ctx *ctx, const ssv_batch_t *b);
+int ssv_getsv_scan_tiles(ssv_ctx *ctx, int64_t *tiles, int64_t *of);
 int ssv_getsv_prime(ssv_ctx *ctx, const ssv_batch_t *b, int32_t *sufficient);
 int ssv_getsv_finish(ssv_ctx *ctx, int32_t *counts,
                      const ssv_interval *ranges, int64_t n_ranges, uint64_t *range_sum,
diff --git a/seeksv_amd/_abi.py b/seeksv_amd/_abi.py
--- a/seeksv_amd/_abi.py
+++ b/seeksv_amd/_abi.py
@@ -347,6 +347,7 @@
         lib.ssv_isize_finish.argtypes = [V, C.POINTER(C.c_int64), C.POINTER(C.c_int32), C.POINTER(C.c_int32)]
         lib.ssv_getsv_begin.argtypes = [V, C.POINTER(GetsvParams)]
         lib.ssv_getsv_scan.argtypes = [V, C.POINTER(Batch)]
+        lib.ssv_getsv_scan_tiles.argtypes = [V, C.POINTER(C.c_int64), C.POINTER(C.c_int64)]
         lib.ssv_getsv_finish.argtypes = [V, V, V, C.c_int64, V, V, C.c_int64, V, C.POINTER(C.c_int32)]
         lib.ssv_bamdec_begin.argtypes = [V, C.c_int32, C.c_uint64]
         lib.ssv_bamdec_staging.argtypes = [V, C.c_int, C.c_size_t, C.POINTER(V)]
diff --git a/seeksv_amd/csrc/bamdec_api.inc b/seeksv_amd/csrc/bamdec_api.inc
--- a/seeksv_amd/csrc/bamdec_api.inc
+++ b/seeksv_amd/csrc/bamdec_api.inc
@@ -360,7 +360,7 @@
 		hipLaunchKernelGGL(ssv::k_record_seqs, dim3((unsigned)std::min<int64_t>((n * 16 + BLOCK - 1) / BLOCK, 2048)), dim3(BLOCK), 0, st, P<uint8_t>(d.stream), P<uint64_t>(d.rec_off),
 		                   col.n_cigar, col.seq_bytes, col.seq_off, P<uint32_t>(d.seq_list), sm + 10, col.seqqual, col.xc);
 		hipLaunchKernelGGL(ssv::k_raw_copy, dim3((unsigned)((n + BLOCK - 1) / BLOCK)), dim3(BLOCK), 0, st, P<uint8_t>(d.stream), P<uint64_t>(d.rec_off), n, P<uint32_t>(d.raw_bytes), P<uint64_t>(d.raw_off), P<uint8_t>(d.raw));
-		CHECK(d.tl.launch(c, st, col.tid, col.flag, n, d.prev_tid, sm + 2, reinterpret_cast<int32_t *>(sm + 3), sm + 11));
+		CHECK(d.tl.launch(c, st, col.tid, col.pos, col.flag, n, d.prev_tid, sm + 2, reinterpret_cast<int32_t *>(sm + 3), sm + 11));
 	}
 	HIPCHECK(c, hipMemcpyAsync(d.h_small.p, d.small.p, 64, hipMemcpyDeviceToHost, st));
 	HIPCHECK(c, hipStreamSynchronize(st));
diff --git a/seeksv_amd/csrc/bamdec_kernels.h b/seeksv_amd/csrc/bamdec_kernels.h
--- a/seeksv_amd/csrc/bamdec_kernels.h
+++ b/seeksv_amd/csrc/bamdec_kernels.h
@@ -592,7 +592,9 @@
 struct TidRun { uint32_t index; int32_t tid; };
 constexpr int32_t TID_NONE = INT32_MIN;
 
-__global__ __launch_bounds__(BLOCK) void k_tid_raw_runs(const int32_t *__restrict__ tid, int64_t n, TidRun *__restrict__ runs, uint32_t cap, uint32_t *__restrict__ count)
+constexpr uint32_t DESCENT_CAP = 15;
+__global__ __launch_bounds__(BLOCK) void k_tid_raw_runs(const int32_t *__restrict__ tid, const int32_t *__restrict__ pos, int64_t n, TidRun *__restrict__ runs, uint32_t cap,
+                                                       uint32_t *__restrict__ count, uint32_t *__restrict__ descents)
 {
 	const int64_t i = (int64_t)blockIdx.x * BLOCK + threadIdx.x;
 	if (i >= n) return;
@@ -600,6 +602,9 @@
 	if (i == 0 || tid[i - 1] != t) {
 		const uint32_t k = atomicAdd(count, 1u);
 		if (k < cap) { runs[k].index = (uint32_t)i; runs[k].tid = t; }
+	} else if (pos[i] < pos[i - 1]) {
+		const uint32_t k = atomicAdd(descents, 1u);
+		if (k < DESCENT_CAP) descents[1 + k] = (uint32_t)i;
 	}
 }
 
diff --git a/seeksv_amd/csrc/getsv_api.inc b/seeksv_amd/csrc/getsv_api.inc
--- a/seeksv_amd/csrc/getsv_api.inc
+++ b/seeksv_amd/csrc/getsv_api.inc
@@ -11,6 +11,9 @@
 	int64_t diff_len = 0;
 	DBuf djunc, counts, wtid, wbeg, wend, woff, diff, tilemap, tile_win, tile_junc, ctgoff, maxdepth, span;
 	DBuf q_tid, q_out64;
+	DBuf scan_mask, scan_blocks, scan_list, scan_list_n;
+	int64_t last_ntiles = 0;
+	bool last_by_range = false;
 	DBuf dense_list, cap_flags, cap_deep, cap_carry, cap_ring, cap_ring_tmp, cap_tail[2][4];
 	int32_t cap_tail_n = 0, cap_tail_cur = 0, cap_ring_mask = 0;
 	HBuf h_q;
@@ -21,13 +24,17 @@
 	memset(&R, 0, sizeof(R));
 	if (!b->tid_runs || b->n_tid_runs <= 0 || b->n_tid_runs > RUN_MAX || getenv("SSV_NO_TID_RUNS")) return SSV_OK;
 	const int64_t k = b->n_tid_runs;
+	bool same_twice = false;
 	if (b->tid_runs[0].first != 0) { c->err = "tid_runs must start at record 0"; return SSV_E_ARG; }
 	for (int64_t i = 0; i < k; ++i) {
 		if (i && b->tid_runs[i].first <= b->tid_runs[i - 1].first) { c->err = "tid_runs must be strictly increasing"; return SSV_E_ARG; }
 		if (b->tid_runs[i].first >= b->n) { c->err = "tid_runs reach past the batch"; return SSV_E_ARG; }
 		R.first[i] = b->tid_runs[i].first; R.tid[i] = b->tid_runs[i].tid;
+		if (b->tid_runs[i].pad == 1) R.sorted |= 1ull << i;
+		if (i && R.tid[i] == R.tid[i - 1]) same_twice = true;
 	}
 	R.first[k] = b->n; R.n = (int32_t)k;
+	if (same_twice) R.sorted = 0;
 	return SSV_OK;
 }
 
@@ -169,10 +176,12 @@
 		CHECK(ensure_host(c, c->h_counters, sizeof(ClipCounters)));
 		HIPCHECK(c, hipMemsetAsync(c->counters.p, 0, sizeof(ClipCounters), c->st));
 		k_verify_runs<<<(unsigned)std::min<int64_t>(256 * 8, (d.n + BLOCK * 4 - 1) / (BLOCK * 4)), BLOCK, 0, c->st>>>(d.tid, d.n, a.runs, &P<ClipCounters>(c->counters)->n_cand);
+		if (a.runs.sorted) k_verify_sorted<<<(unsigned)std::min<int64_t>(256 * 8, (d.n + BLOCK - 1) / BLOCK), BLOCK, 0, c->st>>>(d.pos, d.n, a.runs, &P<ClipCounters>(c->counters)->n_new);
 		HIPCHECK(c, hipGetLastError());
 		HIPCHECK(c, hipMemcpyAsync(c->h_counters.p, c->counters.p, sizeof(ClipCounters), hipMemcpyDeviceToHost, c->st));
 		HIPCHECK(c, hipStreamSynchronize(c->st));
-		const unsigned long long badrec = P<ClipCounters>(c->h_counters)->n_cand;
+		const unsigned long long badrec = P<ClipCounters>(c->h_counters)->n_cand, badpos = P<ClipCounters>(c->h_counters)->n_new;
+		if (badpos && !badrec) { c->err = "a tid run stated as position-sorted is not: pos falls at record " + std::to_string(badpos - 1) + " (SSV_VERIFY_RUNS)"; return SSV_E_ARG; }
 		if (badrec) { c->err = "tid_runs disagree with the tid column at record " + std::to_string(badrec - 1) + " (SSV_VERIFY_RUNS)"; return SSV_E_ARG; }
 	}
 	a.b = d; a.tilemap = P<uint8_t>(G.tilemap); a.tile_win = P<uint32_t>(G.tile_win); a.tile_junc = P<uint32_t>(G.tile_junc); a.ctg_tile_off = P<int64_t>(G.ctgoff); a.n_targets = G.p.n_targets;
@@ -195,6 +204,14 @@
 	ClipCounters *hc = P<ClipCounters>(c->h_counters);
 	ClipCounters *dc = P<ClipCounters>(c->counters);
 	GetsvStage g;
+	const char *scan_env = getenv("SSV_GETSV_SCAN");
+	const bool by_range = a.runs.n > 0 && a.runs.sorted != 0 && d.n >= CS_TILE && ntiles < (1ll << 28) && !(scan_env && !strcmp(scan_env, "stream"));
+	const int64_t list_blocks = (ntiles + BLOCK - 1) / BLOCK;
+	G.last_by_range = by_range; G.last_ntiles = ntiles;
+	if (by_range) {
+		CHECK(ensure(c, G.scan_mask, (size_t)ntiles + 16)); CHECK(ensure(c, G.scan_blocks, (size_t)list_blocks * 4)); CHECK(ensure(c, G.scan_list, (size_t)ntiles * 4));
+		CHECK(ensure(c, G.scan_list_n, 16));
+	}
 	for (int attempt = 0;; ++attempt) {
 		const int64_t block_cap = (c->stage_cap + grid - 1) / grid;
 		CHECK(ensure(c, c->stage, (size_t)block_cap * grid * 4));
@@ -204,7 +221,13 @@
 		g.dense_list = nullptr; g.dense_n = nullptr; g.n_cand = &dc->n_cand;
 		{
 			ProfScope ps(c, P_GETSV_SCAN, d.n);
-			if (a.runs.n > 0 && d.n >= CS_TILE) k_getsv_scan_runs<<<grid, BLOCK, 0, c->st>>>(a, g);
+			if (by_range) {
+				if (attempt == 0) {
+					k_scan_list_count<<<(unsigned)list_blocks, BLOCK, 0, c->st>>>(a, ntiles, P<uint8_t>(G.scan_mask), P<uint32_t>(c->tile_cnt), P<uint32_t>(G.scan_blocks));
+					k_scan_list_emit<<<(unsigned)list_blocks, BLOCK, 0, c->st>>>(P<uint8_t>(G.scan_mask), ntiles, P<uint32_t>(G.scan_blocks), P<uint32_t>(G.scan_list), P<uint32_t>(G.scan_list_n));
+				}
+				k_getsv_scan_list<<<grid, BLOCK, 0, c->st>>>(a, g, P<uint32_t>(G.scan_list), P<uint32_t>(G.scan_list_n));
+			} else if (a.runs.n > 0 && d.n >= CS_TILE) k_getsv_scan_runs<<<grid, BLOCK, 0, c->st>>>(a, g);
 			else k_getsv_scan<<<grid, BLOCK, 0, c->st>>>(a, g);
 		}
 		HIPCHECK(c, hipGetLastError());
@@ -227,6 +250,20 @@
 	}
 	HIPCHECK(c, hipGetLastError());
 	if (a.n_win > 0) CHECK(cap_launches(c, a, d, ntiles, 0));
+	return SSV_OK;
+}
+
+int ssv_getsv_scan_tiles(ssv_ctx *c, int64_t *tiles, int64_t *of)
+{
+	if (!c || !tiles || !of) return SSV_E_ARG;
+	ssv_getsv_state &G = *c->getsv;
+	HIPCHECK(c, hipSetDevice(c->device));
+	*of = G.last_ntiles; *tiles = -1;
+	if (!G.last_by_range) return SSV_OK;
+	CHECK(ensure_host(c, c->h_totals, 64));
+	HIPCHECK(c, hipMemcpyAsync(c->h_totals.p, G.scan_list_n.p, 4, hipMemcpyDeviceToHost, c->st));
+	HIPCHECK(c, hipStreamSynchronize(c->st));
+	*tiles = (int64_t)*P<uint32_t>(c->h_totals);
 	return SSV_OK;
 }
 
diff --git a/seeksv_amd/csrc/getsv_kernels.h b/seeksv_amd/csrc/getsv_kernels.h
--- a/seeksv_amd/csrc/getsv_kernels.h
+++ b/seeksv_amd/csrc/getsv_kernels.h
@@ -2,6 +2,7 @@
 
 #include "clip_kernels.h"
 #include "common.h"
+#include "getsv_ranges.h"
 
 namespace ssv {
 
@@ -100,6 +101,7 @@
 	int32_t n;
 	int32_t tid[RUN_MAX];
 	int64_t first[RUN_MAX + 1];
+	uint64_t sorted;
 };
 
 struct GetsvArgs {
@@ -262,13 +264,9 @@
 	if (w >= n_win) return;
 	const int tid = win_tid[w];
 	if (tid < 0 || tid >= n_targets) return;
-	int64_t p0 = (int64_t)win_beg[w] - span, p1 = (int64_t)win_end[w] - 1;
-	if (p1 < 0) return;
-	if (p0 < 0) p0 = 0;
 	const int64_t base = ctg_tile_off[tid], ntile = ctg_tile_off[tid + 1] - base;
-	int64_t t0 = p0 >> TILE_SHIFT, t1 = p1 >> TILE_SHIFT;
-	if (t0 >= ntile) return;
-	if (t1 >= ntile) t1 = ntile - 1;
+	int64_t t0, t1;
+	if (!gr_window_tiles(win_beg[w], win_end[w], span, ntile, &t0, &t1)) return;
 	for (int64_t t = t0; t <= t1; ++t) {
 		const int col = (int)(t << TILE_SHIFT) + 1;
 		int64_t lo = 0, hi = n_win;
@@ -289,13 +287,9 @@
 	if (k >= n_junc) return;
 	const int tid = junc[k].up_tid;
 	if (tid < 0 || tid >= n_targets) return;
-	int64_t p0 = (int64_t)junc[k].beg - span, p1 = (int64_t)junc[k].end - 1;
-	if (p1 < 0) return;
-	if (p0 < 0) p0 = 0;
 	const int64_t base = ctg_tile_off[tid], ntile = ctg_tile_off[tid + 1] - base;
-	int64_t t0 = p0 >> TILE_SHIFT, t1 = p1 >> TILE_SHIFT;
-	if (t0 >= ntile) return;
-	if (t1 >= ntile) t1 = ntile - 1;
+	int64_t t0, t1;
+	if (!gr_window_tiles(junc[k].beg, junc[k].end, span, ntile, &t0, &t1)) return;
 	for (int64_t t = t0; t <= t1; ++t) {
 		const int64_t want = (t << TILE_SHIFT) - (int64_t)wmax;
 		int64_t lo = 0, hi = n_junc;
@@ -371,6 +365,14 @@
 			while (k + 1 < runs.n && runs.first[k + 1] <= i) ++k;
 			if (tid[i] != runs.tid[k]) atomicMax(bad, (unsigned long long)(i + 1));
 		}
+	}
+}
+
+__global__ __launch_bounds__(BLOCK) void k_verify_sorted(const int32_t *__restrict__ pos, int64_t n, RunTab runs, unsigned long long *bad)
+{
+	for (int64_t i = (int64_t)blockIdx.x * BLOCK + threadIdx.x + 1; i < n; i += (int64_t)gridDim.x * BLOCK) {
+		const int r = gr_run_of(runs.first, runs.n, i);
+		if (((runs.sorted >> r) & 1ull) && runs.first[r] < i && pos[i] < pos[i - 1]) atomicMax(bad, (unsigned long long)(i + 1));
 	}
 }
 
@@ -571,6 +573,143 @@
 			step(tile, pq[j], pq[(j + 1) % NB], pq[(j + CS_AHEAD) % NB], tmq[j], tmq[(j + 1) % NB]);
 			tile += gridDim.x;
 		}
+	}
+	if (g.n_cand && threadIdx.x == 0 && cursor) atomicAdd(g.n_cand, (unsigned long long)cursor);
+	if (cap_seen && a.cap_flag && lane_id() == 0) *a.cap_flag = 1;
+}
+
+
+__global__ __launch_bounds__(BLOCK) void k_scan_list_count(GetsvArgs a, int64_t ntiles, uint8_t *__restrict__ mask8, uint32_t *__restrict__ tile_cnt, uint32_t *__restrict__ block_cnt)
+{
+	const int64_t t = (int64_t)blockIdx.x * BLOCK + threadIdx.x;
+	uint32_t m = 0;
+	if (t < ntiles) {
+		int run;
+		m = gr_forced_mask(a.runs.first, a.runs.n, a.runs.sorted, a.b.n, t, &run);
+		const int tid = run >= 0 ? a.runs.tid[run] : -1;
+		if (!m && tid >= 0 && tid < a.n_targets) {
+			const int64_t base = a.ctg_tile_off[tid];
+			m = gr_tile_mask(a.b.pos, t, a.runs.first[run + 1], a.tilemap + base, a.ctg_tile_off[tid + 1] - base);
+		}
+		mask8[t] = (uint8_t)m;
+		tile_cnt[t] = 0;
+		if (a.cap_flag) {
+			bool seen = false;
+#pragma unroll
+			for (int h = 0; h < 2; ++h) {
+				const int64_t i = (t << GR_SCAN_SHIFT) + h * (1 << (GR_SCAN_SHIFT - 1)), j = i + (1 << GR_SCAN_SHIFT);
+				if (j >= a.b.n) continue;
+				const int r = gr_run_of(a.runs.first, a.runs.n, i);
+				if (a.runs.first[r + 1] > j && ((a.runs.sorted >> r) & 1ull) && a.runs.tid[r] >= 0 && a.b.pos[j] - a.b.pos[i] <= a.cap_span) seen = true;
+			}
+			if (seen) *a.cap_flag = 1;
+		}
+	}
+	const int cnt = __syncthreads_count(m != 0);
+	if (threadIdx.x == 0) block_cnt[blockIdx.x] = (uint32_t)cnt;
+}
+
+__global__ __launch_bounds__(BLOCK) void k_scan_list_emit(const uint8_t *__restrict__ mask8, int64_t ntiles, const uint32_t *__restrict__ block_cnt, uint32_t *__restrict__ list, uint32_t *__restrict__ n_list)
+{
+	__shared__ uint32_t s_before[WAVES_PER_BLOCK], s_w[WAVES_PER_BLOCK];
+	uint32_t part = 0, before, total;
+	for (uint32_t j = threadIdx.x; j < blockIdx.x; j += BLOCK) part += block_cnt[j];
+	block_exclusive_sum<uint32_t>(part, s_before, &before);
+	const int64_t t = (int64_t)blockIdx.x * BLOCK + threadIdx.x;
+	const uint32_t m = t < ntiles ? mask8[t] : 0u;
+	const uint32_t at = block_exclusive_sum<uint32_t>(m ? 1u : 0u, s_w, &total);
+	if (m) list[before + at] = (uint32_t)t << 4 | m;
+	if (blockIdx.x == gridDim.x - 1 && threadIdx.x == 0) *n_list = before + total;
+}
+
+__global__ __launch_bounds__(BLOCK) void k_getsv_scan_list(GetsvArgs a, GetsvStage g, const uint32_t *__restrict__ list, const uint32_t *__restrict__ n_list)
+{
+	__shared__ uint64_t lds[2][WAVES_PER_BLOCK];
+	const DevBatch &b = a.b;
+	uint32_t cursor = 0;
+	int parity = 0;
+	const int64_t region = (int64_t)blockIdx.x * g.block_cap;
+	const int last_tid = a.n_targets - 1;
+	const uint32_t nl = scalar_load(n_list);
+	bool cap_seen = false;
+	auto load = [&](uint32_t e, int4 (&q)[CS_SUB]) -> uint32_t {
+		const uint32_t en = list[e];
+		const int64_t tile = en >> 4;
+		const int64_t t0 = tile * CS_TILE + (int64_t)threadIdx.x * CS_ITEMS;
+		const bool whole = (tile + 1) * CS_TILE <= b.n;
+#pragma unroll
+		for (int sub = 0; sub < CS_SUB; ++sub) {
+			const int64_t i0 = t0 + (int64_t)sub * (BLOCK * CS_ITEMS);
+			if (!((en >> sub) & 1u)) q[sub] = make_int4(-1, -1, -1, -1);
+			else if (whole) q[sub] = stream_load_i4(b.pos + i0);
+			else {
+				int pp[CS_ITEMS];
+#pragma unroll
+				for (int k = 0; k < CS_ITEMS; ++k) pp[k] = i0 + k < b.n ? b.pos[i0 + k] : -1;
+				q[sub] = make_int4(pp[0], pp[1], pp[2], pp[3]);
+			}
+		}
+		return en;
+	};
+	int4 p4[CS_SUB], np4[CS_SUB];
+	uint32_t en = 0, nen = 0;
+	if (blockIdx.x < nl) en = load(blockIdx.x, p4);
+	for (uint32_t e = blockIdx.x; e < nl; e += gridDim.x, parity ^= 1) {
+		if (e + gridDim.x < nl) nen = load(e + gridDim.x, np4);
+		const int64_t tile = en >> 4;
+		const int64_t t0 = tile * CS_TILE + (int64_t)threadIdx.x * CS_ITEMS;
+		const int run = tile_run_tid(a.runs, tile, b.n);
+		uint32_t mask = 0;
+		int pmin = 0x7fffffff, pmax = -1;
+#pragma unroll
+		for (int sub = 0; sub < CS_SUB; ++sub) if ((en >> sub) & 1u) {
+			pmin = min(pmin, min(min(p4[sub].x, p4[sub].y), min(p4[sub].z, p4[sub].w)));
+			pmax = max(pmax, max(max(p4[sub].x, p4[sub].y), max(p4[sub].z, p4[sub].w)));
+		}
+		const bool uniform = run >= 0 && run <= last_tid && __all(pmin >= 0);
+		int wmin = 0, wmax = 0;
+		if (uniform) {
+			const int wpmin = -wave_max(-pmin), wpmax = wave_max(pmax);
+			wmin = wpmin >> TILE_SHIFT; wmax = wpmax >> TILE_SHIFT;
+			cap_seen = cap_seen || ((en & GR_FULL) == GR_FULL && wpmax - wpmin <= a.cap_span);
+		}
+		if (uniform && wmax - wmin < WAVE) {
+			const int64_t lo = scalar_load(a.ctg_tile_off + run), hi = scalar_load(a.ctg_tile_off + run + 1);
+			const int64_t mine = lo + wmin + lane_id();
+			const uint64_t interesting = __ballot(mine < hi && a.tilemap[mine < hi ? mine : hi - 1] != 0);
+			if (interesting) {
+#pragma unroll
+				for (int sub = 0; sub < CS_SUB; ++sub) if ((en >> sub) & 1u) {
+					const int pos[CS_ITEMS] = {p4[sub].x, p4[sub].y, p4[sub].z, p4[sub].w};
+#pragma unroll
+					for (int k = 0; k < CS_ITEMS; ++k)
+						mask |= ((uint32_t)(interesting >> ((pos[k] >> TILE_SHIFT) - wmin)) & 1u) << (sub * CS_ITEMS + k);
+				}
+			}
+		} else {
+#pragma unroll
+			for (int sub = 0; sub < CS_SUB; ++sub) if ((en >> sub) & 1u) {
+				const int pos[CS_ITEMS] = {p4[sub].x, p4[sub].y, p4[sub].z, p4[sub].w};
+#pragma unroll
+				for (int k = 0; k < CS_ITEMS; ++k) {
+					const int64_t i = t0 + (int64_t)sub * (BLOCK * CS_ITEMS) + k;
+					const int tid = run >= 0 ? run : (i < b.n ? a.runs.tid[gr_run_of(a.runs.first, a.runs.n, i)] : -1);
+					const int tc = tid < 0 ? 0 : (tid > last_tid ? last_tid : tid);
+					const int64_t lo = a.ctg_tile_off[tc], hi = a.ctg_tile_off[tc + 1];
+					int64_t t = lo + ((pos[k] < 0 ? 0 : pos[k]) >> TILE_SHIFT);
+					const bool valid = tid >= 0 && tid <= last_tid && pos[k] >= 0 && t < hi;
+					t = t < hi ? t : hi - 1;
+					if (valid && a.tilemap[t] != 0) mask |= 1u << (sub * CS_ITEMS + k);
+				}
+			}
+		}
+		uint64_t packed = 0;
+#pragma unroll
+		for (int sub = 0; sub < CS_SUB; ++sub) packed |= (uint64_t)__popc((mask >> (sub * CS_ITEMS)) & ((1u << CS_ITEMS) - 1u)) << (16 * sub);
+		stage_tile_candidates<CS_ITEMS, true>(mask, packed, tile, t0, lds, parity, cursor, region, g.block_cap, g.tile_cnt, g.tile_off, g.stage, g.overflow);
+#pragma unroll
+		for (int sub = 0; sub < CS_SUB; ++sub) p4[sub] = np4[sub];
+		en = nen;
 	}
 	if (g.n_cand && threadIdx.x == 0 && cursor) atomicAdd(g.n_cand, (unsigned long long)cursor);
 	if (cap_seen && a.cap_flag && lane_id() == 0) *a.cap_flag = 1;
diff --git a/seeksv_amd/csrc/getsv_ranges.h b/seeksv_amd/csrc/getsv_ranges.h
--- /dev/null
+++ b/seeksv_amd/csrc/getsv_ranges.h
@@ -0,0 +1,73 @@
+#pragma once
+
+#include <stdint.h>
+
+#if defined(__HIPCC__)
+#define SSV_GR_FN __host__ __device__ inline
+#else
+#define SSV_GR_FN inline
+#endif
+
+namespace ssv {
+
+constexpr int GR_TILE_SHIFT = 9;
+constexpr int GR_SUB_SHIFT = 10;
+constexpr int GR_SUBS_SHIFT = 2;
+constexpr int GR_SCAN_SHIFT = GR_SUB_SHIFT + GR_SUBS_SHIFT;
+constexpr uint32_t GR_FULL = (1u << (1 << GR_SUBS_SHIFT)) - 1u;
+constexpr int GR_PROBE_MAX = 64;
+
+SSV_GR_FN bool gr_window_tiles(int32_t beg, int32_t end, int32_t span, int64_t ntile, int64_t *t0, int64_t *t1)
+{
+	int64_t p0 = (int64_t)beg - span, p1 = (int64_t)end - 1;
+	if (p1 < 0) return false;
+	if (p0 < 0) p0 = 0;
+	*t0 = p0 >> GR_TILE_SHIFT; *t1 = p1 >> GR_TILE_SHIFT;
+	if (*t0 >= ntile) return false;
+	if (*t1 >= ntile) *t1 = ntile - 1;
+	return *t0 <= *t1;
+}
+
+SSV_GR_FN bool gr_span_marked(const uint8_t *marks, int64_t ntile, int32_t lo, int32_t hi)
+{
+	if (hi < 0) return false;
+	const int64_t t0 = (lo < 0 ? 0 : lo) >> GR_TILE_SHIFT;
+	int64_t t1 = hi >> GR_TILE_SHIFT;
+	if (t0 >= ntile) return false;
+	if (t1 >= ntile) t1 = ntile - 1;
+	if (t1 - t0 >= GR_PROBE_MAX) return true;
+	bool any = false;
+	for (int64_t t = t0; t <= t1; ++t) any = any || marks[t] != 0;
+	return any;
+}
+
+SSV_GR_FN uint32_t gr_tile_mask(const int32_t *pos, int64_t tile, int64_t run_end, const uint8_t *marks, int64_t ntile)
+{
+	const int64_t t0 = tile * ((int64_t)1 << GR_SCAN_SHIFT), next = t0 + ((int64_t)1 << GR_SCAN_SHIFT);
+	int32_t p[(1 << GR_SUBS_SHIFT) + 1];
+	for (int s = 0; s < 1 << GR_SUBS_SHIFT; ++s) p[s] = pos[t0 + s * ((int64_t)1 << GR_SUB_SHIFT)];
+	p[1 << GR_SUBS_SHIFT] = pos[next < run_end ? next : next - 1];
+	uint32_t m = 0;
+	for (int s = 0; s < 1 << GR_SUBS_SHIFT; ++s) if (gr_span_marked(marks, ntile, p[s], p[s + 1])) m |= 1u << s;
+	return m;
+}
+
+SSV_GR_FN int gr_run_of(const int64_t *first, int n_runs, int64_t i)
+{
+	int lo = 0, hi = n_runs - 1;
+	while (lo < hi) { const int m = (lo + hi + 1) >> 1; if (first[m] <= i) lo = m; else hi = m - 1; }
+	return lo;
+}
+
+SSV_GR_FN uint32_t gr_forced_mask(const int64_t *first, int n_runs, uint64_t sorted, int64_t n, int64_t tile, int *run)
+{
+	const int64_t t0 = tile * ((int64_t)1 << GR_SCAN_SHIFT), t1 = t0 + ((int64_t)1 << GR_SCAN_SHIFT);
+	*run = -1;
+	if (t1 > n) return GR_FULL;
+	const int r = gr_run_of(first, n_runs, t0);
+	if (first[r + 1] < t1) return GR_FULL;
+	*run = r;
+	return (sorted >> r) & 1u ? 0u : GR_FULL;
+}
+
+}
diff --git a/seeksv_amd/csrc/samdec_api.inc b/seeksv_amd/csrc/samdec_api.inc
--- a/seeksv_amd/csrc/samdec_api.inc
+++ b/seeksv_amd/csrc/samdec_api.inc
@@ -247,7 +247,7 @@
 			                                                                                                                                col.l_qseq, col.seq_off, col.seqqual, errw);
 		if (raw_total) k_sam_raw<<<grid_for(n, BLOCK), BLOCK, 0, st>>>(tx, P<uint32_t>(d.sep), P<uint32_t>(d.nlidx), n, col, srt.raw_bytes, P<uint64_t>(d.raw_off), P<uint8_t>(d.raw), errw);
 		HIPCHECK(c, hipGetLastError());
-		CHECK(d.tl.launch(c, st, col.tid, col.flag, n, d.prev_tid, sm + 12, reinterpret_cast<int32_t *>(sm + 13), sm + 14));
+		CHECK(d.tl.launch(c, st, col.tid, col.pos, col.flag, n, d.prev_tid, sm + 12, reinterpret_cast<int32_t *>(sm + 13), sm + 14));
 	} else {
 		k_sam_fields<<<grid_for(n, BLOCK), BLOCK, 0, st>>>(tx, P<uint32_t>(d.sep), P<uint32_t>(d.nlidx), n, T, col, lines, reinterpret_cast<int32_t *>(sm + 8), errw);
 		k_sam_seqqual<<<(unsigned)std::min<int64_t>((n + WAVES_PER_BLOCK - 1) / WAVES_PER_BLOCK, 8192), BLOCK, 0, st>>>(tx, P<uint32_t>(d.sep), P<uint32_t>(d.nlidx), n, col.l_qseq, col.seq_off,
diff --git a/seeksv_amd/csrc/seeksv_hip.hip b/seeksv_amd/csrc/seeksv_hip.hip
--- a/seeksv_amd/csrc/seeksv_hip.hip
+++ b/seeksv_amd/csrc/seeksv_hip.hip
@@ -537,6 +537,7 @@
 
 struct TidLists {
 	static constexpr uint32_t RUN_CAP = 1u << 16, RAW_RUN_CAP = 64;
+	static constexpr size_t RAW_BYTES = (size_t)RAW_RUN_CAP * sizeof(ssv::TidRun) + (ssv::DESCENT_CAP + 1) * 4;
 	DBuf tile_last, tile_prev, runs, raw_runs;
 	HBuf h_raw_runs, h_runs;
 	std::vector<ssv_tid_run> tid_runs;
@@ -545,17 +546,19 @@
 		const size_t n_tiles = (size_t)((n + BLOCK - 1) / BLOCK);
 		CHECK(ensure(c, tile_last, grown(n_tiles * 4, grow))); CHECK(ensure(c, tile_prev, grown(n_tiles * 4, grow)));
 		CHECK(ensure(c, runs, grown((size_t)RUN_CAP * sizeof(ssv::TidRun), grow)));
-		CHECK(ensure(c, raw_runs, grown((size_t)RAW_RUN_CAP * sizeof(ssv::TidRun), grow)));
-		return ensure_host(c, h_raw_runs, (size_t)RAW_RUN_CAP * sizeof(ssv::TidRun));
-	}
-	int launch(ssv_ctx *c, hipStream_t st, const int32_t *tid, const uint16_t *flag, int64_t n, int32_t prev_tid, uint32_t *n_runs, int32_t *last_tid, uint32_t *n_raw_runs)
+		CHECK(ensure(c, raw_runs, grown(RAW_BYTES, grow)));
+		return ensure_host(c, h_raw_runs, RAW_BYTES);
+	}
+	int launch(ssv_ctx *c, hipStream_t st, const int32_t *tid, const int32_t *pos, const uint16_t *flag, int64_t n, int32_t prev_tid, uint32_t *n_runs, int32_t *last_tid, uint32_t *n_raw_runs)
 	{
 		const int64_t n_tiles = (n + BLOCK - 1) / BLOCK;
 		hipLaunchKernelGGL(ssv::k_tid_tile_last, dim3((unsigned)n_tiles), dim3(BLOCK), 0, st, tid, flag, n, P<int32_t>(tile_last));
 		hipLaunchKernelGGL(ssv::k_tid_tile_carry, dim3(1), dim3(WAVE), 0, st, P<int32_t>(tile_last), n_tiles, prev_tid, P<int32_t>(tile_prev), last_tid);
 		hipLaunchKernelGGL(ssv::k_tid_runs, dim3((unsigned)n_tiles), dim3(BLOCK), 0, st, tid, flag, n, P<int32_t>(tile_prev), P<ssv::TidRun>(runs), RUN_CAP, n_runs);
-		hipLaunchKernelGGL(ssv::k_tid_raw_runs, dim3((unsigned)n_tiles), dim3(BLOCK), 0, st, tid, n, P<ssv::TidRun>(raw_runs), RAW_RUN_CAP, n_raw_runs);
-		HIPCHECK(c, hipMemcpyAsync(h_raw_runs.p, raw_runs.p, (size_t)RAW_RUN_CAP * sizeof(ssv::TidRun), hipMemcpyDeviceToHost, st));
+		uint32_t *descents = reinterpret_cast<uint32_t *>(P<ssv::TidRun>(raw_runs) + RAW_RUN_CAP);
+		HIPCHECK(c, hipMemsetAsync(descents, 0, (ssv::DESCENT_CAP + 1) * 4, st));
+		hipLaunchKernelGGL(ssv::k_tid_raw_runs, dim3((unsigned)n_tiles), dim3(BLOCK), 0, st, tid, pos, n, P<ssv::TidRun>(raw_runs), RAW_RUN_CAP, n_raw_runs, descents);
+		HIPCHECK(c, hipMemcpyAsync(h_raw_runs.p, raw_runs.p, RAW_BYTES, hipMemcpyDeviceToHost, st));
 		return SSV_OK;
 	}
 	int fetch(ssv_ctx *c, hipStream_t st, uint32_t n_runs)
@@ -580,6 +583,15 @@
 		const ssv::TidRun *r = P<ssv::TidRun>(h_raw_runs);
 		for (uint32_t k = 0; k < nr; ++k) tid_runs.push_back(ssv_tid_run{(int64_t)r[k].index, r[k].tid, 0});
 		std::sort(tid_runs.begin(), tid_runs.end(), [](const ssv_tid_run &a, const ssv_tid_run &b) { return a.first < b.first; });
+		const uint32_t *descents = reinterpret_cast<const uint32_t *>(r + RAW_RUN_CAP);
+		if (descents[0] <= ssv::DESCENT_CAP) {
+			for (ssv_tid_run &t : tid_runs) t.pad = 1;
+			for (uint32_t k = 0; k < descents[0]; ++k) {
+				size_t q = 0;
+				while (q + 1 < tid_runs.size() && tid_runs[q + 1].first <= (int64_t)descents[1 + k]) ++q;
+				tid_runs[q].pad = 0;
+			}
+		}
 		out->tid_runs = tid_runs.data(); out->n_tid_runs = (int64_t)nr;
 	}
 };
diff --git a/seeksv_amd/device.py b/seeksv_amd/device.py
--- a/seeksv_amd/device.py
+++ b/seeksv_amd/device.py
@@ -346,6 +346,11 @@
         b, keep = self._as_batch(batch)
         self._check(self._lib.ssv_getsv_scan(self._h, C.byref(b)), "ssv_getsv_scan")
 
+    def getsv_scan_tiles(self):
+        t, of = C.c_int64(), C.c_int64()
+        self._check(self._lib.ssv_getsv_scan_tiles(self._h, C.byref(t), C.byref(of)), "ssv_getsv_scan_tiles")
+        return t.value, of.value
+
     def getsv_finish(self, ranges, points):
         r = np.ascontiguousarray(ranges, dtype=_abi.INTERVAL_DTYPE)
         q = np.ascontiguousarray(points, dtype=_abi.INTERVAL_DTYPE)
diff --git a/seeksv_amd/synth.py b/seeksv_amd/synth.py
--- a/seeksv_amd/synth.py
+++ b/seeksv_amd/synth.py
@@ -295,10 +295,14 @@
             starts = np.concatenate(([0], ch)).astype(np.int64)
             runs = np.zeros(len(starts), _abi.TID_RUN_DTYPE)
             runs["first"], runs["tid"] = starts, tt[torch.from_numpy(starts).to(dev)].cpu().numpy()
+            pp = t["pos"]
+            fall = (torch.nonzero((pp[1:] < pp[:-1]) & (tt[1:] == tt[:-1])).flatten() + 1).cpu().numpy()
+            runs["pad"] = 1
+            runs["pad"][np.searchsorted(starts, fall, side="right") - 1] = 0
             arrays["tid_runs"] = runs
         elif n == 1:
             runs = np.zeros(1, _abi.TID_RUN_DTYPE)
-            runs["tid"] = int(t["tid"][0].item())
+            runs["tid"], runs["pad"] = int(t["tid"][0].item()), 1
             arrays["tid_runs"] = runs
         b, _ = _abi.make_batch(arrays, mem=_abi.MEM_DEVICE | (_abi.MEM_PERSISTENT if persistent else 0), n=n)
         return b, t
```

Result: no change. 68.63 billion (-0.2%).
